# FofanovLab/mtsv_tools

Hardware: AMD Instinct MI355X
Metric: reads/sec (whole node), 150bp reads vs MG-index (higher is better)
Workload: dtype u32/i16

## Files before the change

include/mtsv_amd.h:

```cpp
#ifndef MTSV_AMD_H
#define MTSV_AMD_H

#include <stddef.h>
#include <stdint.h>

#ifdef __cplusplus
extern "C" {
#endif

#define MTSV_OK 0
#define MTSV_E_ARG (-1)
#define MTSV_E_IO (-2)
#define MTSV_E_FORMAT (-3)
#define MTSV_E_DEVICE (-4)
#define MTSV_E_LIMIT (-5)
#define MTSV_E_NOMEM (-6)

typedef struct mtsv_index mtsv_index;
typedef struct mtsv_batch mtsv_batch;

typedef struct {
    double edit_rate;
    uint32_t seed_size;
    uint32_t seed_interval;
    double min_seed;
    uint64_t max_hits;
    uint64_t tune_max_hits;
    int64_t max_assignments;
    int64_t max_candidates;
} mtsv_params;

typedef struct {
    uint64_t read;
    uint32_t tax_id;
    uint32_t gi;
    uint32_t edit;
    uint8_t strand;
    uint8_t _pad[3];
    uint64_t offset;
} mtsv_hit;

typedef struct {
    uint64_t n;
    uint64_t n_bins;
    uint32_t occ_k;
    uint64_t sa_s;
    uint64_t file_bytes;
    uint64_t device_bytes;
    uint32_t kmer_k;
    uint32_t sa_full;
} mtsv_index_info_t;

#define MTSV_N_STAGES 8
typedef struct {
    float stage_ms[MTSV_N_STAGES];
    uint64_t n_reads;
    uint64_t n_seed_slots;
    uint64_t n_seed_hits;
    uint64_t lf_steps;
    uint64_t n_candidates;
    uint64_t n_verified;
    uint64_t window_bytes;
    uint64_t n_hits;
    uint64_t n_passes;
    uint64_t n_rounds;
    uint64_t n_lanes;
    uint64_t sw_cell_pairs;
    float sw_prefilter_ms;
    float sw_sweep_ms;
    uint64_t n_sw_passed;
    float sw_diag_ms;
    float sw_bound_ms;
    float edit_ms;
    uint64_t myers_columns;
    uint64_t n_sw_bound_refuted;
} mtsv_batch_stats;

const char *mtsv_last_error(void);
const char *mtsv_version(void);
void mtsv_params_default(mtsv_params *p);

int mtsv_device_count(void);

int mtsv_index_load(const char *path, mtsv_index **out);
int mtsv_index_build(uint64_t n_seqs, const uint32_t *tax_ids, const uint32_t *gis,
                     const uint8_t *const *seqs, const uint64_t *seq_lens, uint32_t occ_k,
                     uint64_t sa_s, int n_threads, mtsv_index **out);
int mtsv_index_build_fasta(const char *fasta_path, uint32_t occ_k, uint64_t sa_s, int n_threads,
                           mtsv_index **out);
int mtsv_set_build_device(int hip_device);
int mtsv_index_write(const mtsv_index *ix, const char *path);
int mtsv_index_info(const mtsv_index *ix, mtsv_index_info_t *info);
void mtsv_index_free(mtsv_index *ix);

#define MTSV_DEV_DEFAULT 0u
#define MTSV_DEV_SAMPLED_SA_ONLY 1u
#define MTSV_DEV_NO_KMER_TABLE 2u
int mtsv_index_to_device(mtsv_index *ix, int hip_device, uint32_t flags);

int mtsv_bin_batch(mtsv_index *ix, int hip_device, const uint8_t *bases, const uint64_t *read_off,
                   uint64_t n_reads, const mtsv_params *params, mtsv_hit **hits, uint64_t *n_hits);
void mtsv_hits_free(mtsv_hit *hits);
void *mtsv_host_alloc(size_t bytes);
void mtsv_host_free(void *p);
int mtsv_host_register(void *p, size_t bytes);
int mtsv_host_unregister(void *p);
int mtsv_bin_batch_multi(mtsv_index *ix, const int *devices, int n_devices, const uint8_t *bases,
                         const uint64_t *read_off, uint64_t n_reads, const mtsv_params *params,
                         mtsv_hit **hits, uint64_t *n_hits);
int mtsv_bin_batch_chunks(mtsv_index *const *chunks, const int *devices, int n_chunks,
                          const uint8_t *bases, const uint64_t *read_off, uint64_t n_reads,
                          const mtsv_params *params, mtsv_hit **hits, uint64_t *n_hits);
uint64_t mtsv_bin_batch_workspace_reads(uint64_t n_reads);

int mtsv_batch_create(mtsv_index *ix, int hip_device, uint64_t max_reads, uint64_t max_bases,
                      uint64_t max_hits_ws, mtsv_batch **out);
int mtsv_batch_create_lanes(mtsv_index *ix, int hip_device, uint64_t max_reads, uint64_t max_bases,
                            uint64_t max_hits_ws, int lanes, mtsv_batch **out);
int mtsv_batch_reserve_host(mtsv_batch *b, uint64_t n_reads, uint64_t n_bases, uint32_t warm_read_len);
#define MTSV_VERIFY_REFERENCE 0
#define MTSV_VERIFY_EDIT_FIRST 1
int mtsv_batch_set_verify_mode(mtsv_batch *b, int mode);
int mtsv_set_default_verify_mode(int mode);
int mtsv_batch_upload(mtsv_batch *b, const uint8_t *bases, const uint64_t *read_off,
                      uint64_t n_reads);
int mtsv_batch_run(mtsv_batch *b, const mtsv_params *params);
int mtsv_batch_run_host(mtsv_batch *b, const uint8_t *bases, const uint64_t *read_off,
                        uint64_t n_reads, const mtsv_params *params);
int mtsv_batch_run_host_parts(mtsv_batch *b, int n_parts, const uint8_t *const *bases, const uint64_t *const *read_off,
                              const uint64_t *n_reads, const mtsv_params *params);
int mtsv_batch_stats_get(const mtsv_batch *b, mtsv_batch_stats *st);

typedef struct {
    uint32_t tax_id;
    uint32_t _pad;
    uint64_t only_hit, only_best, tied_best, not_best;
} mtsv_taxon_stats;
int mtsv_batch_set_taxa_report(mtsv_batch *b, int on);
int mtsv_batch_taxa_report(mtsv_batch *b, mtsv_taxon_stats **rows, uint64_t *n_rows, uint64_t *total_reads,
                           float *device_ms, int reset);
int mtsv_merge_taxa_reports(const mtsv_taxon_stats *a, uint64_t n_a, const mtsv_taxon_stats *b, uint64_t n_b,
                            mtsv_taxon_stats **out, uint64_t *n_out);
int mtsv_format_taxa_report(const mtsv_taxon_stats *rows, uint64_t n_rows, uint64_t total_reads, char **out,
                            uint64_t *out_len);

#define MTSV_MATCH_OFF 0
#define MTSV_MATCH_WITH_HITS 1
#define MTSV_MATCH_ONLY 2
int mtsv_batch_set_match_flags(mtsv_batch *b, int mode);
int mtsv_batch_match_flags(mtsv_batch *b, uint64_t **words, uint64_t *n_reads, uint64_t *n_matched);
int mtsv_batch_download(mtsv_batch *b, mtsv_hit **hits, uint64_t *n_hits);
void mtsv_batch_free(mtsv_batch *b);

int mtsv_format_results(const mtsv_hit *hits, uint64_t n_hits, const char *ids,
                        const uint64_t *id_off, uint64_t n_reads, int long_format, char **out,
                        uint64_t *out_len);
void mtsv_free(void *p);

uint8_t mtsv_pack_bases(uint8_t *dst, const uint8_t *src, uint64_t first_offset, uint64_t n, uint8_t prev_code);
int mtsv_host_pack_threads(void);

int mtsv_synth_index(uint64_t seed, uint32_t n_taxa, uint32_t gis_per_taxon, uint64_t seq_len,
                     uint32_t occ_k, uint64_t sa_s, int n_threads, mtsv_index **out);
int mtsv_synth_reads(const mtsv_index *ix, uint64_t seed, uint64_t n_reads, uint32_t read_len,
                     uint8_t *bases, uint64_t *read_off);

#ifdef __cplusplus
}
#endif
#endif
```

mtsv_tools_amd/_lib.py:

```python
import ctypes as C
import os

import numpy as np

_HERE = os.path.dirname(os.path.abspath(__file__))


def lib_path():
    return os.environ.get("MTSV_AMD_LIB") or os.path.join(_HERE, "libmtsv_amd.so")


class MtsvError(RuntimeError):
    def __init__(self, code, msg):
        super().__init__(f"mtsv error {code}: {msg}")
        self.code = code


E_ARG, E_IO, E_FORMAT, E_DEVICE, E_LIMIT, E_NOMEM = -1, -2, -3, -4, -5, -6
MATCH_OFF, MATCH_WITH_HITS, MATCH_ONLY = 0, 1, 2


class Params(C.Structure):
    _fields_ = [("edit_rate", C.c_double), ("seed_size", C.c_uint32), ("seed_interval", C.c_uint32),
                ("min_seed", C.c_double), ("max_hits", C.c_uint64), ("tune_max_hits", C.c_uint64),
                ("max_assignments", C.c_int64), ("max_candidates", C.c_int64)]


class IndexInfo(C.Structure):
    _fields_ = [("n", C.c_uint64), ("n_bins", C.c_uint64), ("occ_k", C.c_uint32),
                ("sa_s", C.c_uint64), ("file_bytes", C.c_uint64), ("device_bytes", C.c_uint64),
                ("kmer_k", C.c_uint32), ("sa_full", C.c_uint32)]


N_STAGES = 8
STAGE_NAMES = ("search", "thin_scan", "expand", "locate", "coalesce", "verify", "gather", "total")


class BatchStats(C.Structure):
    _fields_ = [("stage_ms", C.c_float * N_STAGES), ("n_reads", C.c_uint64),
                ("n_seed_slots", C.c_uint64), ("n_seed_hits", C.c_uint64), ("lf_steps", C.c_uint64),
                ("n_candidates", C.c_uint64), ("n_verified", C.c_uint64),
                ("window_bytes", C.c_uint64), ("n_hits", C.c_uint64), ("n_passes", C.c_uint64),
                ("n_rounds", C.c_uint64), ("n_lanes", C.c_uint64), ("sw_cell_pairs", C.c_uint64), ("sw_prefilter_ms", C.c_float),
                ("sw_sweep_ms", C.c_float), ("n_sw_passed", C.c_uint64), ("sw_diag_ms", C.c_float), ("sw_bound_ms", C.c_float),
                ("edit_ms", C.c_float), ("myers_columns", C.c_uint64), ("n_sw_bound_refuted", C.c_uint64)]

    def as_dict(self):
        d = {n: (float(getattr(self, n)) if t is C.c_float else int(getattr(self, n))) for n, t in self._fields_[1:]}
        d["stage_ms"] = {STAGE_NAMES[i]: float(self.stage_ms[i]) for i in range(N_STAGES)}
        return d


HIT_DTYPE = np.dtype({"names": ["read", "tax_id", "gi", "edit", "strand", "offset"],
                      "formats": ["<u8", "<u4", "<u4", "<u4", "u1", "<u8"],
                      "offsets": [0, 8, 12, 16, 20, 24], "itemsize": 32})

TAXON_STATS_DTYPE = np.dtype({"names": ["tax_id", "only_hit", "only_best", "tied_best", "not_best"],
                              "formats": ["<u4", "<u8", "<u8", "<u8", "<u8"],
                              "offsets": [0, 8, 16, 24, 32], "itemsize": 40})

EXPORTS = [
    "mtsv_last_error", "mtsv_version", "mtsv_params_default", "mtsv_device_count",
    "mtsv_index_load", "mtsv_index_build", "mtsv_index_build_fasta", "mtsv_index_write",
    "mtsv_index_info", "mtsv_index_free", "mtsv_set_build_device", "mtsv_index_to_device", "mtsv_bin_batch",
    "mtsv_hits_free", "mtsv_batch_create", "mtsv_batch_upload", "mtsv_batch_run", "mtsv_batch_run_host", "mtsv_batch_run_host_parts",
    "mtsv_batch_stats_get", "mtsv_batch_set_verify_mode", "mtsv_batch_download", "mtsv_batch_free", "mtsv_format_results",
    "mtsv_free", "mtsv_synth_index", "mtsv_synth_reads", "mtsv_bin_batch_workspace_reads",
    "mtsv_bin_batch_multi", "mtsv_bin_batch_chunks", "mtsv_set_default_verify_mode",
    "mtsv_host_alloc", "mtsv_host_free", "mtsv_host_register", "mtsv_host_unregister",
    "mtsv_batch_create_lanes", "mtsv_batch_reserve_host", "mtsv_pack_bases", "mtsv_host_pack_threads",
    "mtsv_batch_set_taxa_report", "mtsv_batch_taxa_report", "mtsv_merge_taxa_reports", "mtsv_format_taxa_report",
    "mtsv_batch_set_match_flags", "mtsv_batch_match_flags",
]

_lib = None


def lib():
    global _lib
    if _lib is None:
        p = lib_path()
        if not os.path.exists(p):
            raise MtsvError(E_DEVICE, f"{p} is missing: run `make -C mtsv_tools_amd/csrc` "
                                      "(or __graft_entry__.build()); there is no fallback path")
        L = C.CDLL(p)
        vp, u64, u32, i32 = C.c_void_p, C.c_uint64, C.c_uint32, C.c_int
        L.mtsv_last_error.restype = C.c_char_p
        L.mtsv_version.restype = C.c_char_p
        L.mtsv_params_default.argtypes = [C.POINTER(Params)]
        L.mtsv_index_load.argtypes = [C.c_char_p, C.POINTER(vp)]
        L.mtsv_index_build.argtypes = [u64, vp, vp, vp, vp, u32, u64, i32, C.POINTER(vp)]
        L.mtsv_index_build_fasta.argtypes = [C.c_char_p, u32, u64, i32, C.POINTER(vp)]
        L.mtsv_index_write.argtypes = [vp, C.c_char_p]
        L.mtsv_index_info.argtypes = [vp, C.POINTER(IndexInfo)]
        L.mtsv_index_free.argtypes = [vp]
        L.mtsv_index_free.restype = None
        L.mtsv_index_to_device.argtypes = [vp, i32, u32]
        L.mtsv_bin_batch.argtypes = [vp, i32, vp, vp, u64, C.POINTER(Params), C.POINTER(vp),
                                     C.POINTER(u64)]
        L.mtsv_hits_free.argtypes = [vp]
        L.mtsv_hits_free.restype = None
        L.mtsv_bin_batch_multi.argtypes = [vp, vp, i32, vp, vp, u64, C.POINTER(Params), C.POINTER(vp), C.POINTER(u64)]
        L.mtsv_bin_batch_chunks.argtypes = [vp, vp, i32, vp, vp, u64, C.POINTER(Params), C.POINTER(vp), C.POINTER(u64)]
        L.mtsv_bin_batch_workspace_reads.argtypes = [u64]
        L.mtsv_bin_batch_workspace_reads.restype = u64
        L.mtsv_batch_create.argtypes = [vp, i32, u64, u64, u64, C.POINTER(vp)]
        L.mtsv_batch_create_lanes.argtypes = [vp, i32, u64, u64, u64, i32, C.POINTER(vp)]
        L.mtsv_batch_reserve_host.argtypes = [vp, u64, u64, u32]
        L.mtsv_pack_bases.argtypes = [vp, vp, u64, u64, C.c_uint8]
        L.mtsv_pack_bases.restype = C.c_uint8
        L.mtsv_batch_upload.argtypes = [vp, vp, vp, u64]
        L.mtsv_batch_run.argtypes = [vp, C.POINTER(Params)]
        L.mtsv_batch_run_host.argtypes = [vp, vp, vp, u64, C.POINTER(Params)]
        L.mtsv_batch_run_host_parts.argtypes = [vp, i32, vp, vp, vp, C.POINTER(Params)]
        L.mtsv_batch_set_verify_mode.argtypes = [vp, i32]
        L.mtsv_batch_stats_get.argtypes = [vp, C.POINTER(BatchStats)]
        L.mtsv_batch_download.argtypes = [vp, C.POINTER(vp), C.POINTER(u64)]
        L.mtsv_batch_free.argtypes = [vp]
        L.mtsv_batch_free.restype = None
        L.mtsv_format_results.argtypes = [vp, u64, C.c_char_p, vp, u64, i32, C.POINTER(vp),
                                          C.POINTER(u64)]
        L.mtsv_free.argtypes = [vp]
        L.mtsv_free.restype = None
        L.mtsv_synth_index.argtypes = [u64, u32, u32, u64, u32, u64, i32, C.POINTER(vp)]
        L.mtsv_synth_reads.argtypes = [vp, u64, u64, u32, vp, vp]
        L.mtsv_host_alloc.argtypes = [C.c_size_t]
        L.mtsv_host_alloc.restype = vp
        L.mtsv_host_free.argtypes = [vp]
        L.mtsv_host_free.restype = None
        L.mtsv_host_register.argtypes = [vp, C.c_size_t]
        L.mtsv_host_unregister.argtypes = [vp]
        L.mtsv_batch_set_taxa_report.argtypes = [vp, i32]
        L.mtsv_batch_taxa_report.argtypes = [vp, C.POINTER(vp), C.POINTER(u64), C.POINTER(u64), C.POINTER(C.c_float), i32]
        L.mtsv_merge_taxa_reports.argtypes = [vp, u64, vp, u64, C.POINTER(vp), C.POINTER(u64)]
        L.mtsv_format_taxa_report.argtypes = [vp, u64, u64, C.POINTER(vp), C.POINTER(u64)]
        L.mtsv_batch_set_match_flags.argtypes = [vp, i32]
        L.mtsv_batch_match_flags.argtypes = [vp, C.POINTER(vp), C.POINTER(u64), C.POINTER(u64)]
        _lib = L
    return _lib


def _check(rc):
    if rc != 0:
        raise MtsvError(rc, lib().mtsv_last_error().decode(errors="replace"))


def version():
    return lib().mtsv_version().decode()


def device_count():
    return lib().mtsv_device_count()


def bin_batch_multi(index, devices, bases, read_off, params=None):
    params = params or default_params()
    bases = np.ascontiguousarray(bases, dtype=np.uint8)
    read_off = np.ascontiguousarray(read_off, dtype=np.uint64)
    dev = (C.c_int * len(devices))(*devices)
    out, n = C.c_void_p(), C.c_uint64()
    _check(lib().mtsv_bin_batch_multi(index.h, dev, len(devices), bases.ctypes.data, read_off.ctypes.data,
                                      len(read_off) - 1, C.byref(params), C.byref(out), C.byref(n)))
    return _hits_from(out, n.value)


def bin_batch_chunks(indexes, devices, bases, read_off, params=None):
    params = params or default_params()
    bases = np.ascontiguousarray(bases, dtype=np.uint8)
    read_off = np.ascontiguousarray(read_off, dtype=np.uint64)
    dev = (C.c_int * len(devices))(*devices)
    hs = (C.c_void_p * len(indexes))(*[ix.h for ix in indexes])
    out, n = C.c_void_p(), C.c_uint64()
    _check(lib().mtsv_bin_batch_chunks(hs, dev, len(indexes), bases.ctypes.data, read_off.ctypes.data,
                                       len(read_off) - 1, C.byref(params), C.byref(out), C.byref(n)))
    return _hits_from(out, n.value)


class HostBuffer:

    def __init__(self, nbytes):
        self.ptr = lib().mtsv_host_alloc(nbytes)
        if not self.ptr:
            raise MtsvError(E_DEVICE, lib().mtsv_last_error().decode(errors="replace"))
        self.array = np.ctypeslib.as_array((C.c_uint8 * max(1, nbytes)).from_address(self.ptr))[:nbytes]

    def close(self):
        if self.ptr:
            self.array = None
            lib().mtsv_host_free(self.ptr)
            self.ptr = None


def pack_bases(bases, first_offset=0, prev_code=0):
    bases = np.ascontiguousarray(bases, dtype=np.uint8)
    n = len(bases)
    out = np.zeros(((first_offset + n + 1) >> 1) - (first_offset >> 1) + 1, dtype=np.uint8)
    last = lib().mtsv_pack_bases(out.ctypes.data, bases.ctypes.data, first_offset, n, prev_code)
    return out[:-1], last


def host_register(arr):
    _check(lib().mtsv_host_register(arr.ctypes.data, arr.nbytes))


def host_unregister(arr):
    _check(lib().mtsv_host_unregister(arr.ctypes.data))


def bin_batch_slice_reads(n_reads):
    return int(lib().mtsv_bin_batch_workspace_reads(n_reads))


def set_build_device(device):
    lib().mtsv_set_build_device.argtypes = [C.c_int]
    _check(lib().mtsv_set_build_device(device))


def default_params(**over):
    p = Params()
    lib().mtsv_params_default(C.byref(p))
    names = {f[0] for f in Params._fields_}
    for k, v in over.items():
        if k not in names:
            raise AttributeError(f"no such parameter: {k}")
        setattr(p, k, -1 if v is None else v)
    return p


def _hits_from(ptr, n):
    try:
        if n == 0:
            return np.zeros(0, dtype=HIT_DTYPE)
        raw = (C.c_ubyte * (n * HIT_DTYPE.itemsize)).from_address(ptr.value)
        return np.frombuffer(raw, dtype=HIT_DTYPE).copy()
    finally:
        lib().mtsv_hits_free(ptr)


class MGIndex:

    def __init__(self, handle):
        self.h = handle

    @classmethod
    def load(cls, path):
        h = C.c_void_p()
        _check(lib().mtsv_index_load(os.fsencode(path), C.byref(h)))
        return cls(h)

    @classmethod
    def build(cls, entries, occ_k=64, sa_s=32, threads=4):
        entries = list(entries)
        n = len(entries)
        tax = np.array([e[0] for e in entries], dtype=np.uint32)
        gi = np.array([e[1] for e in entries], dtype=np.uint32)
        bufs = [C.create_string_buffer(bytes(e[2]), max(len(e[2]), 1)) for e in entries]
        ptrs = (C.c_void_p * max(n, 1))(*[C.addressof(b) for b in bufs])
        lens = np.array([len(e[2]) for e in entries], dtype=np.uint64)
        h = C.c_void_p()
        _check(lib().mtsv_index_build(n, tax.ctypes.data, gi.ctypes.data, ptrs, lens.ctypes.data,
                                      occ_k, sa_s, threads, C.byref(h)))
        return cls(h)

    @classmethod
    def build_fasta(cls, path, occ_k=64, sa_s=32, threads=4):
        h = C.c_void_p()
        _check(lib().mtsv_index_build_fasta(os.fsencode(path), occ_k, sa_s, threads, C.byref(h)))
        return cls(h)

    @classmethod
    def synth(cls, seed, n_taxa, gis_per_taxon, seq_len, occ_k=64, sa_s=32, threads=8):
        h = C.c_void_p()
        _check(lib().mtsv_synth_index(seed, n_taxa, gis_per_taxon, seq_len, occ_k, sa_s, threads,
                                      C.byref(h)))
        return cls(h)

    def write(self, path):
        _check(lib().mtsv_index_write(self.h, os.fsencode(path)))

    def info(self):
        i = IndexInfo()
        _check(lib().mtsv_index_info(self.h, C.byref(i)))
        return {n: int(getattr(i, n)) for n, _ in i._fields_}

    def to_device(self, device=0, flags=0):
        _check(lib().mtsv_index_to_device(self.h, device, flags))

    def bin_batch(self, bases, read_off, params=None, device=0):
        params = params or default_params()
        bases = np.ascontiguousarray(bases, dtype=np.uint8)
        read_off = np.ascontiguousarray(read_off, dtype=np.uint64)
        out, n = C.c_void_p(), C.c_uint64()
        _check(lib().mtsv_bin_batch(self.h, device, bases.ctypes.data, read_off.ctypes.data,
                                    len(read_off) - 1, C.byref(params), C.byref(out), C.byref(n)))
        return _hits_from(out, n.value)

    def close(self):
        if self.h is not None and _lib is not None:
            _lib.mtsv_index_free(self.h)
        self.h = None

    def __del__(self):
        try:
            self.close()
        except Exception:
            pass


class Batch:

    def __init__(self, index, device, max_reads, max_bases, max_hits_ws=0, lanes=0):
        self.index = index
        self.h = C.c_void_p()
        _check(lib().mtsv_batch_create_lanes(index.h, device, max_reads, max_bases, max_hits_ws, lanes,
                                             C.byref(self.h)))

    def reserve_host(self, n_reads, n_bases, warm_read_len=0):
        _check(lib().mtsv_batch_reserve_host(self.h, n_reads, n_bases, warm_read_len))

    def upload(self, bases, read_off):
        bases = np.ascontiguousarray(bases, dtype=np.uint8)
        read_off = np.ascontiguousarray(read_off, dtype=np.uint64)
        _check(lib().mtsv_batch_upload(self.h, bases.ctypes.data, read_off.ctypes.data,
                                       len(read_off) - 1))

    def set_verify_mode(self, mode):
        _check(lib().mtsv_batch_set_verify_mode(self.h, mode))

    def run(self, params=None):
        params = params or default_params()
        _check(lib().mtsv_batch_run(self.h, C.byref(params)))

    def run_host(self, bases, read_off, params=None):
        params = params or default_params()
        bases = np.ascontiguousarray(bases, dtype=np.uint8)
        read_off = np.ascontiguousarray(read_off, dtype=np.uint64)
        _check(lib().mtsv_batch_run_host(self.h, bases.ctypes.data, read_off.ctypes.data, len(read_off) - 1,
                                         C.byref(params)))

    def run_host_parts(self, parts, params=None):
        params = params or default_params()
        keep = [(np.ascontiguousarray(b, dtype=np.uint8), np.ascontiguousarray(o, dtype=np.uint64)) for b, o in parts]
        k = len(keep)
        bp = (C.c_void_p * k)(*[b.ctypes.data for b, _ in keep])
        op = (C.c_void_p * k)(*[o.ctypes.data for _, o in keep])
        nr = (C.c_uint64 * k)(*[len(o) - 1 for _, o in keep])
        _check(lib().mtsv_batch_run_host_parts(self.h, k, bp, op, nr, C.byref(params)))

# ... 101 lines not shown
```

mtsv_tools_amd/csrc/batch.hip:

```cpp
#include <atomic>
#include <chrono>
#include <cmath>
#include <condition_variable>
#include <exception>
#include <mutex>
#include <thread>
#include <cstdio>
#include <cstdlib>
#include <cstring>
#include <stdexcept>
#include <vector>

#include "../../include/mtsv_amd.h"
#include "batch.hpp"
#include "kernels.hpp"

namespace mtsv {

namespace {
template <class F>
void parallel_ranges(uint64_t n, F f) {
    static const int max_nt = [] {
        const char* e = getenv("MTSV_COPY_THREADS");
        return e ? std::max(1, std::min(16, atoi(e))) : 4;
    }();
    const int nt = std::min(max_nt, n >= (32ull << 20) ? 4 : n >= (4ull << 20) ? 2 : 1);
    if (nt == 1) return f(0, n);
    std::vector<std::thread> th;
    const uint64_t chunk = ((n + nt - 1) / nt + 4095) & ~4095ull;
    for (int k = 0; k < nt; k++) {
        uint64_t a = std::min(n, chunk * k), b = std::min(n, chunk * (k + 1));
        if (a < b) th.emplace_back([=] { f(a, b); });
    }
    for (auto& t : th) t.join();
}
double now_s() { return std::chrono::duration<double>(std::chrono::steady_clock::now().time_since_epoch()).count(); }
void parallel_copy(uint8_t* dst, const uint8_t* src, uint64_t n) {
    parallel_ranges(n, [=](uint64_t a, uint64_t b) { memcpy(dst + a, src + a, b - a); });
}

template <class T>
void dev_alloc(T** p, uint64_t count, uint64_t* bytes) {
    uint64_t b = std::max<uint64_t>(count, 1) * sizeof(T);
    HIP_CHECK(hipMalloc((void**)p, b));
    *bytes += b;
}
}

bool host_pinned(const void* p, uint64_t bytes) {
    if (!p || !bytes) return false;
    for (const uint8_t* q : {(const uint8_t*)p, (const uint8_t*)p + bytes - 1}) {
        hipPointerAttribute_t at;
        memset(&at, 0, sizeof at);
        if (hipPointerGetAttributes(&at, q) != hipSuccess) {
            (void)hipGetLastError();
            return false;
        }
        if (at.type != hipMemoryTypeHost) return false;
    }
    return true;
}

void* host_pinned_alloc(uint64_t bytes) {
    void* p = nullptr;
    if (hipHostMalloc(&p, bytes ? bytes : 1, hipHostMallocPortable) != hipSuccess) {
        (void)hipGetLastError();
        return nullptr;
    }
    return p;
}
void host_pinned_free(void* p) {
    if (p && hipHostFree(p) != hipSuccess) (void)hipGetLastError();
}
bool host_pinned_register(void* p, uint64_t bytes) {
    if (hipHostRegister(p, bytes, hipHostRegisterPortable) == hipSuccess) return true;
    (void)hipGetLastError();
    return false;
}
bool host_pinned_unregister(void* p) {
    if (hipHostUnregister(p) == hipSuccess) return true;
    (void)hipGetLastError();
    return false;
}


int g_default_verify_mode = MTSV_VERIFY_REFERENCE;

constexpr uint64_t kLaneMinReads = 32768;
constexpr uint64_t kChunkMaxReads = 4ull << 20;

Batch::Batch(mtsv_index* ix_, DeviceIndex* di_, uint64_t max_reads_, uint64_t max_bases_, uint64_t hit_cap_, Batch* parent_, int lanes_)
    : ix(ix_), di(di_), max_reads(max_reads_), max_bases(max_bases_), hit_cap(hit_cap_), parent(parent_) {
    if (max_reads == 0) max_reads = 1;
    if (max_reads > 0x7fffffffull) throw std::runtime_error("limit: more than 2^31 reads in one batch");
    if (max_bases >= 0xffffffffull) throw std::runtime_error("limit: 4 GiB of bases or more in one batch");
    const uint64_t hit_cap_user = hit_cap;
    if (!parent) {
        n_lanes = 3;
        if (lanes_ > 0) n_lanes = std::min(8, lanes_);
        else if (const char* e = getenv("MTSV_LANES")) n_lanes = std::max(1, std::min(8, atoi(e)));
        if (max_reads < (uint64_t)n_lanes * kLaneMinReads) n_lanes = 1;
    }
    ws_reads = (max_reads + n_lanes - 1) / n_lanes;
    if (!parent && n_lanes > 1) {
        uint64_t cmax = kChunkMaxReads;
        if (const char* e = getenv("MTSV_CHUNK")) cmax = std::max<uint64_t>(kLaneMinReads, strtoull(e, nullptr, 10));
        ws_reads = std::min(ws_reads, cmax);
    }
    if (hit_cap == 0) hit_cap = std::max<uint64_t>(1ull << 20, 32 * ws_reads);
    if (hit_cap > 0xfffffff0ull) hit_cap = 0xfffffff0ull;
    hits_cap = std::max<uint64_t>(1ull << 20, 16 * ws_reads);
    if (const char* e = getenv("MTSV_HITS_CAP")) hits_cap = std::max<uint64_t>(1024, strtoull(e, nullptr, 10));
    HIP_CHECK(hipSetDevice(di->device));
    HIP_CHECK(hipStreamCreateWithFlags(&stream, hipStreamNonBlocking));
    const uint64_t ns = 2 * ws_reads;
    if (!parent) {
        dev_alloc(&d_bases, max_bases + 64, &bytes);
        dev_alloc(&d_read_off, max_reads + 1, &bytes);
        dev_alloc(&d_codes, max_bases + 64, &bytes);
    }
    dev_alloc(&d_strand_hits, ns + 1, &bytes);
    dev_alloc(&d_strand_nseeds, ns, &bytes);
    dev_alloc(&d_strand_off, ns + 1, &bytes);
    dev_alloc(&d_strand_ncand, ns, &bytes);
    dev_alloc(&d_strand_nout, ns + 1, &bytes);
    dev_alloc(&d_heavy_list, 2 * ns, &bytes);
    dev_alloc(&d_out_off, ns + 1, &bytes);
    dev_alloc(&d_tile_sums, (uint64_t)scan_tiles((uint32_t)ns) + 1, &bytes);
    dev_alloc(&d_counters, kCounters, &bytes);
    alloc_hit_workspace();
    dev_alloc(&d_hits, hits_cap, &bytes);
    HIP_CHECK(hipHostMalloc((void**)&h_counters, kCounters * sizeof(uint64_t), hipHostMallocMapped));
    if (const char* e = getenv("MTSV_SW")) sw_pairs = strcmp(e, "packed") != 0;
    if (const char* e = getenv("MTSV_SW_DIAG")) sw_diag = atoi(e) != 0;
    if (const char* e = getenv("MTSV_SW_PREPASS")) sw_prepass = atoi(e) != 0;
    if (const char* e = getenv("MTSV_SW_TOP")) sw_top = atoi(e) != 0;
    if (const char* e = getenv("MTSV_SW_BOUND")) sw_bound = atoi(e) != 0;
    if (const char* e = getenv("MTSV_SW_FUSED")) sw_fused = atoi(e) != 0;
    verify_mode = g_default_verify_mode;
    if (const char* e = getenv("MTSV_VERIFY")) verify_mode = !strcmp(e, "edit_first") ? 1 : 0;
    for (auto& e : ev) HIP_CHECK(hipEventCreate(&e));
    for (int k = 1; k < n_lanes; k++) {
        extra.emplace_back(new Batch(ix, di, ws_reads, 0, hit_cap_user, this));
        bytes += extra.back()->bytes;
    }
}

Batch::~Batch() {
    extra.clear();
    (void)hipSetDevice(di->device);
    (void)hipStreamSynchronize(stream);
    for (void* p : {(void*)d_bases, (void*)d_read_off, (void*)d_seed_lo, (void*)d_seed_cnt, (void*)d_seed_pre, (void*)d_strand_hits,
                    (void*)d_strand_nseeds, (void*)d_strand_off, (void*)d_strand_ncand, (void*)d_worklist,
                    (void*)d_strand_nout, (void*)d_out_off, (void*)d_tile_sums, (void*)d_counters, (void*)d_hit_row,
                    (void*)d_hit_ref, (void*)d_hit_q, (void*)d_hit_key, (void*)d_cand_tmp, (void*)d_cand, (void*)d_out,
                    (void*)d_hits, (void*)d_cand_next, (void*)d_cand_status, (void*)d_heavy_list})
        (void)hipFree(p);
    (void)hipFree(d_codes);
    (void)hipFree(d_strip);
    (void)hipFree(d_planes);
    (void)hipFree(report.d_taxa);
    (void)hipFree(report.d_counts);
    for (auto& e : report_ev)
        if (e) (void)hipEventDestroy(e);
    (void)hipFree(match.d_words);
    for (auto& e : match_ev)
        if (e) (void)hipEventDestroy(e);
    if (h_hits_stage) pinned_hits_release(h_hits_stage);
    if (copy_stream2) (void)hipStreamDestroy(copy_stream2);
    if (copy_stream) {
        (void)hipStreamSynchronize(copy_stream);
        (void)hipStreamDestroy(copy_stream);
    }
    for (auto& ar : arena) {
        (void)hipFree(ar.d_bases);
        (void)hipFree(ar.d_packed);
        (void)hipFree(ar.d_off);
    }
    if (h_off_all) (void)hipHostFree(h_off_all);
    for (auto& hs : h_stage)
        if (hs) (void)hipHostFree(hs);
    for (auto& e : chunk_ev) (void)hipEventDestroy(e);
    (void)hipHostFree(h_counters);
    for (auto& e : ev) (void)hipEventDestroy(e);
    (void)hipStreamDestroy(stream);
}

void Batch::alloc_hit_workspace() {
    dev_alloc(&d_hit_row, hit_cap, &bytes);
    dev_alloc(&d_hit_ref, hit_cap, &bytes);
    dev_alloc(&d_hit_q, hit_cap, &bytes);
    dev_alloc(&d_hit_key, hit_cap, &bytes);
    dev_alloc(&d_cand_tmp, 2 * hit_cap, &bytes);
    dev_alloc(&d_cand, hit_cap, &bytes);
    dev_alloc(&d_out, hit_cap, &bytes);
    dev_alloc(&d_cand_next, hit_cap, &bytes);
    dev_alloc(&d_cand_status, hit_cap, &bytes);
    dev_alloc(&d_worklist, hit_cap, &bytes);
}

void Batch::grow_hit_workspace(uint64_t need) {
    if (getenv("MTSV_TRACE")) fprintf(stderr, "[workspace] seed-hit arrays grow %llu -> %llu entries\n", (unsigned long long)hit_cap, (unsigned long long)need);
    HIP_CHECK(hipStreamSynchronize(stream));
    for (void* p : {(void*)d_hit_row, (void*)d_hit_ref, (void*)d_hit_q, (void*)d_hit_key, (void*)d_cand_tmp, (void*)d_cand,
                    (void*)d_out, (void*)d_cand_next, (void*)d_cand_status, (void*)d_worklist})
        (void)hipFree(p);
    d_hit_row = d_hit_ref = d_hit_q = d_cand_next = d_cand_status = d_worklist = nullptr;
    d_hit_key = d_cand_tmp = nullptr;
    d_cand = d_out = nullptr;
    hit_cap = need;
    alloc_hit_workspace();
}

void Batch::upload(const uint8_t* bases, const uint64_t* read_off, uint64_t n) {
    if (n > max_reads) throw std::runtime_error("arg: batch holds more reads than the workspace was created for");
    const uint64_t first = n ? read_off[0] : 0;
    const uint64_t nb = n ? read_off[n] - first : 0;
    if (nb > max_bases) throw std::runtime_error("arg: batch holds more bases than the workspace was created for");
    h_read_off.resize(n + 1);
    max_len = 0;
    for (uint64_t i = 0; i <= n; i++) {
        if (i && read_off[i] < read_off[i - 1]) throw std::runtime_error("arg: read_off is not ascending");
        h_read_off[i] = (uint32_t)(read_off[i] - first);
        if (i) max_len = std::max(max_len, h_read_off[i] - h_read_off[i - 1]);
    }
    if (n == 0) h_read_off[0] = 0;
    HIP_CHECK(hipSetDevice(di->device));
    if (nb) HIP_CHECK(hipMemcpyAsync(d_bases, bases + first, nb, hipMemcpyHostToDevice, stream));
    HIP_CHECK(hipMemcpyAsync(d_read_off, h_read_off.data(), (n + 1) * 4, hipMemcpyHostToDevice, stream));
    HIP_CHECK(hipStreamSynchronize(stream));
    n_reads = n;
    n_hits_total = 0;
    total_hits = 0;
    segments.clear();
}

void Batch::reset_lane() {
    HIP_CHECK(hipSetDevice(di->device));
    memset(&stats, 0, sizeof stats);
    memset(stage_acc, 0, sizeof stage_acc);
    sw_ms_acc = 0;
    sweep_ms_acc = diag_ms_acc = bound_ms_acc = edit_ms_acc = 0;
    sw_passed_acc = 0;
    n_hits_total = 0;
    HIP_CHECK(hipMemsetAsync(d_counters, 0, kCounters * sizeof(uint64_t), stream));
    HIP_CHECK(hipEventRecord(ev[8], stream));
}

void Batch::finish_lane() {
    HIP_CHECK(hipEventRecord(ev[9], stream));
    launch_publish(stream, d_counters, h_counters, kCounters);
    HIP_CHECK(hipStreamSynchronize(stream));
    HIP_CHECK(hipEventElapsedTime(&stage_acc[7], ev[8], ev[9]));
    if (getenv("MTSV_TRACE")) fprintf(stderr, "[lane] last pass: %llu strands of 13..64 seed hits (or more than 4 candidates) to k_coalesce_mid, %llu heavier ones\n",
                                      (unsigned long long)(h_counters[15] & 0xffffffffull), (unsigned long long)(h_counters[1] >> 32));
    if (getenv("MTSV_TRACE")) fprintf(stderr, "[lane] k_coalesce_heavy: %llu strands walked by runs, %llu by the wavefront walk (a run too long)\n",
                                      (unsigned long long)(h_counters[kCtrHeavyWalk] & 0xffffffffull), (unsigned long long)(h_counters[kCtrHeavyWalk] >> 32));
    stats.sw_cell_pairs = h_counters[14];
    stats.sw_prefilter_ms = sw_ms_acc;
    stats.sw_sweep_ms = sweep_ms_acc;
    stats.sw_diag_ms = diag_ms_acc;
    stats.sw_bound_ms = bound_ms_acc;
    stats.edit_ms = edit_ms_acc;
    stats.myers_columns = h_counters[19];
    stats.n_sw_bound_refuted = h_counters[20];
    stats.n_sw_passed = sw_passed_acc + h_counters[21];
    stats.lf_steps = h_counters[2];
    stats.n_candidates = h_counters[3];
    stats.n_verified = h_counters[4];
    stats.window_bytes = h_counters[5];
}

void Batch::begin_run(const mtsv_params& p, uint64_t read_base) {
    if (!(p.edit_rate >= 0.0 && p.edit_rate <= 1.0)) throw std::runtime_error("arg: edit_rate must be within [0, 1]");
    if (!(p.min_seed >= 0.0) || !std::isfinite(p.min_seed)) throw std::runtime_error("arg: min_seed must be finite and >= 0");
    if (p.seed_size == 0 || p.seed_interval == 0) throw std::runtime_error("arg: seed_size and seed_interval must be > 0");
    segments.clear();
    total_hits = 0;
    lanes_used = 1;
    staged_valid = false;
    run_t0 = now_s();
    reset_lane();
    for (auto& l : extra) {
        l->verify_mode = verify_mode;
        l->sw_pairs = sw_pairs;
        l->sw_diag = sw_diag;
        l->sw_prepass = sw_prepass;
        l->sw_top = sw_top;
        l->sw_bound = sw_bound;
        l->sw_fused = sw_fused;
        l->reset_lane();
    }
    if (match.mode != MTSV_MATCH_OFF) {
        const uint64_t need = (n_reads + 63) / 64;
        if (need > match.cap_words || !match.d_words) {
            (void)hipFree(match.d_words);
            match.d_words = nullptr;
            match.cap_words = 0;
            uint64_t b = 0;
            dev_alloc(&match.d_words, need + need / 16 + 1, &b);
            match.cap_words = need + need / 16;
        }
        match.n_reads = n_reads;
        match.call_base = read_base;
        match.ms = 0;
        match.launches = 0;
        HIP_CHECK(hipMemsetAsync(match.d_words, 0, (match.cap_words + 1) * sizeof(uint64_t), stream));
        HIP_CHECK(hipStreamSynchronize(stream));
    }
}

void Batch::end_run() {
    finish_lane();
    for (auto& l : extra) l->finish_lane();
    const double wall_ms = (now_s() - run_t0) * 1e3;
    bool overlapped = false;
    for (auto& l : extra) {
        if (l->stats.n_passes == 0) continue;
        overlapped = true;
        for (int s = 0; s < 7; s++) stage_acc[s] += l->stage_acc[s];
        stats.n_seed_slots += l->stats.n_seed_slots;
        stats.n_seed_hits += l->stats.n_seed_hits;
        stats.n_passes += l->stats.n_passes;
        stats.n_rounds = std::max(stats.n_rounds, l->stats.n_rounds);
        stats.lf_steps += l->stats.lf_steps;
        stats.n_candidates += l->stats.n_candidates;
        stats.n_verified += l->stats.n_verified;
        stats.window_bytes += l->stats.window_bytes;
        stats.sw_cell_pairs += l->stats.sw_cell_pairs;
        stats.sw_prefilter_ms += l->stats.sw_prefilter_ms;
        stats.sw_sweep_ms += l->stats.sw_sweep_ms;
        stats.sw_diag_ms += l->stats.sw_diag_ms;
        stats.sw_bound_ms += l->stats.sw_bound_ms;
        stats.edit_ms += l->stats.edit_ms;
        stats.myers_columns += l->stats.myers_columns;
        stats.n_sw_bound_refuted += l->stats.n_sw_bound_refuted;
        stats.n_sw_passed += l->stats.n_sw_passed;
    }
    if (overlapped) stage_acc[7] = (float)wall_ms;
    for (int s = 0; s < MTSV_N_STAGES; s++) stats.stage_ms[s] = stage_acc[s];
    stats.n_reads = n_reads;
    stats.n_lanes = lanes_used;
    total_hits = 0;
    for (auto& sg : segments) total_hits += sg.count;
    stats.n_hits = total_hits;
}

void Batch::set_taxa_report(bool on) {
    if (parent) throw std::runtime_error("internal: the taxa report belongs to the workspace's owner");
    if (on && match.mode == MTSV_MATCH_ONLY)
        throw std::runtime_error("arg: the taxa report reads gathered hits and MTSV_MATCH_ONLY gathers none (mtsv_batch_set_match_flags)");
    if (on && !report.d_counts) {
        std::vector<uint32_t>& t = report.h_taxa;
        t.clear();
        for (const Bin& b : ix->host.bins) t.push_back(b.tax_id);
        std::sort(t.begin(), t.end());
        t.erase(std::unique(t.begin(), t.end()), t.end());
        if (t.size() >= (1ull << 30)) throw std::runtime_error("limit: taxa report of 2^30 TaxIDs or more");
        report.n_taxa = (uint32_t)t.size();
        uint32_t dense_max = kReportDenseTaxa;
        if (const char* e = getenv("MTSV_REPORT_DENSE_MAX")) dense_max = (uint32_t)std::min<uint64_t>(strtoull(e, nullptr, 10), kReportDenseTaxa);
        report.dense = report.n_taxa <= dense_max;
        if (const char* e = getenv("MTSV_REPORT_HASH_SLOTS")) {
            const uint64_t want = std::min<uint64_t>(std::max<uint64_t>(strtoull(e, nullptr, 10), 16), kReportHashSlots);
            report.hash_slots = 16;
            while (report.hash_slots * 2 <= want) report.hash_slots *= 2;
        }
        report.trace = getenv("MTSV_TRACE") != nullptr;
        if (report.trace)
            fprintf(stderr, "[report] %u taxa: %s tier (dense up to %u taxa, hash table of %u slots)\n", report.n_taxa,
                    report.dense ? "dense" : "hashed", dense_max, report.hash_slots);
        HIP_CHECK(hipSetDevice(di->device));
        uint64_t b = 0;
        dev_alloc(&report.d_taxa, report.n_taxa, &b);
        dev_alloc(&report.d_counts, 4ull * report.n_taxa + 2, &b);
        if (report.n_taxa) HIP_CHECK(hipMemcpyAsync(report.d_taxa, t.data(), t.size() * 4, hipMemcpyHostToDevice, stream));
        HIP_CHECK(hipMemsetAsync(report.d_counts, 0, (4ull * report.n_taxa + 2) * 8, stream));
        HIP_CHECK(hipStreamSynchronize(stream));
    }
    report.on = on;
}

void Batch::taxa_report(std::vector<mtsv_taxon_stats>& rows, uint64_t* total_reads, float* device_ms, bool reset) {
    if (!report.on) throw std::runtime_error("arg: the taxa report of this workspace is not switched on (mtsv_batch_set_taxa_report)");
    HIP_CHECK(hipSetDevice(di->device));
    const uint64_t n = 4ull * report.n_taxa + 2;
    std::vector<uint64_t> c(n);
    HIP_CHECK(hipMemcpyAsync(c.data(), report.d_counts, n * 8, hipMemcpyDeviceToHost, stream));
    if (reset) HIP_CHECK(hipMemsetAsync(report.d_counts, 0, n * 8, stream));
    HIP_CHECK(hipStreamSynchronize(stream));
    rows.clear();
    for (uint32_t k = 0; k < report.n_taxa; k++) {
        const uint64_t* q = &c[4ull * k];
        if (q[0] | q[1] | q[2] | q[3]) rows.push_back(mtsv_taxon_stats{report.h_taxa[k], 0, q[0], q[1], q[2], q[3]});
    }
    *total_reads = c[n - 2];
    std::lock_guard<std::mutex> lk(report.mu);
    *device_ms = report.ms;
    if (report.trace)
        fprintf(stderr, "[report] %llu kernel launches, %.3f ms, %llu atomic adds on the global counters\n", (unsigned long long)report.launches,
                report.ms, (unsigned long long)c[n - 1]);
    if (reset) report.ms = 0, report.launches = 0;
}

void Batch::set_match_flags(int mode) {
    if (parent) throw std::runtime_error("internal: the match flags belong to the workspace's owner");
    if (mode != MTSV_MATCH_OFF && mode != MTSV_MATCH_WITH_HITS && mode != MTSV_MATCH_ONLY) throw std::runtime_error("arg: bad match-flags mode");
    if (mode == MTSV_MATCH_ONLY && report.on)
        throw std::runtime_error("arg: MTSV_MATCH_ONLY gathers no hits and the taxa report of this workspace, which reads them, is on");
    if (mode != MTSV_MATCH_OFF && match.mode == MTSV_MATCH_OFF) match.n_reads = 0;
    match.trace = getenv("MTSV_TRACE") != nullptr;
    match.mode = mode;
}

void Batch::match_flags(std::vector<uint64_t>& words, uint64_t* n_reads_out, uint64_t* n_matched) {
    if (match.mode == MTSV_MATCH_OFF) throw std::runtime_error("arg: the match flags of this workspace are not switched on (mtsv_batch_set_match_flags)");
    const uint64_t nw = (match.n_reads + 63) / 64;
    words.assign(std::max<uint64_t>(nw, 1), 0);
    *n_reads_out = match.n_reads;
    *n_matched = 0;
    if (!match.n_reads) return;
    HIP_CHECK(hipSetDevice(di->device));
    HIP_CHECK(hipMemcpyAsync(words.data(), match.d_words, nw * 8, hipMemcpyDeviceToHost, stream));
    HIP_CHECK(hipMemcpyAsync(n_matched, match.d_words + match.cap_words, 8, hipMemcpyDeviceToHost, stream));
    HIP_CHECK(hipStreamSynchronize(stream));
    std::lock_guard<std::mutex> lk(match.mu);
    if (match.trace)
        fprintf(stderr, "[match] %llu kernel launches, %.3f ms, %llu of %llu reads matched, %llu bytes of flags to the host\n",
                (unsigned long long)match.launches, match.ms, (unsigned long long)*n_matched, (unsigned long long)match.n_reads,
                (unsigned long long)(nw * 8 + 8));
}

void Batch::run(const mtsv_params& p) {
    begin_run(p);
    run_range(p, d_bases, d_codes, d_read_off, h_read_off.data(), n_reads, max_len, 0);
    end_run();
}

void Batch::run_range(const mtsv_params& p, const uint8_t* raw, uint8_t* sb, const uint32_t* so, const uint32_t* h_off, uint64_t n,
                      uint32_t range_max_len, uint64_t read_base) {
    std::vector<Batch*> ls{this};
    for (auto& l : extra) ls.push_back(l.get());
    uint64_t k = n >= ls.size() * kLaneMinReads ? ls.size() : 1;
    uint64_t per_lane = 2;
    if (const char* e = getenv("MTSV_CHUNKS_PER_LANE")) per_lane = std::max(1, atoi(e));
    uint64_t n_chunks = std::max<uint64_t>(k, (n + ws_reads - 1) / ws_reads);
    if (k > 1 && n >= k * per_lane * kLaneMinReads) n_chunks = std::max(n_chunks, k * per_lane);
    std::vector<uint64_t> bound(n_chunks + 1, n);
    bound[0] = 0;
    while (k > 1 && n_chunks >= 2 * k && (double)n / ((double)n_chunks - (double)(k - 1) / 2.0) > (double)ws_reads) n_chunks++;
    bound.assign(n_chunks + 1, n);
    bound[0] = 0;
    if (k > 1 && n_chunks >= 2 * k) {
        const double per0 = (double)n / ((double)n_chunks - (double)(k - 1) / 2.0);
        uint64_t at = 0;
        for (uint64_t c = 0; c < k; c++) {
            at += (uint64_t)(per0 * (double)(c + 1) / (double)k);
            bound[c + 1] = std::min(at, n);
        }
        const uint64_t rest = n - bound[k], m = n_chunks - k;
        for (uint64_t c = 0; c < m; c++) bound[k + c + 1] = bound[k] + rest * (c + 1) / m;
    } else {
        for (uint64_t c = 0; c < n_chunks; c++) bound[c + 1] = n * (c + 1) / n_chunks;
    }
    for (uint64_t c = 0; c < n_chunks; c++)
        if (bound[c + 1] - bound[c] > ws_reads) throw std::runtime_error("arg: range holds more reads than the workspace was created for");
    k = std::min(k, n_chunks);
    lanes_used = std::max<uint64_t>(lanes_used, k);
    std::vector<Segment> segs(n_chunks);
    std::atomic<uint64_t> next{0};
    auto work = [&](Batch* lane) {
        for (;;) {
            const uint64_t c = next.fetch_add(1);
            if (c >= n_chunks) return;
            const uint64_t a = bound[c], b = bound[c + 1];
            const uint64_t before = lane->n_hits_total;
            if (raw) launch_normalise(lane->stream, raw, sb, h_off[a], h_off[b]);
            lane->run_slice(p, sb, so + a, h_off ? h_off + a : nullptr, b - a, range_max_len, read_base + a);
            segs[c] = Segment{lane, before, lane->n_hits_total - before};
        }
    };
    if (k == 1) {
        work(this);
    } else {
        std::vector<std::exception_ptr> errs(k);
        std::vector<std::thread> th;
        for (uint64_t i = 1; i < k; i++)
            th.emplace_back([&, i] {
                try {
                    HIP_CHECK(hipSetDevice(di->device));
                    work(ls[i]);
                } catch (...) {
                    errs[i] = std::current_exception();
                    next.store(n_chunks);
                }
            });
        try {
            work(this);
        } catch (...) {
            errs[0] = std::current_exception();
            next.store(n_chunks);
        }
        for (auto& t : th) t.join();
        for (auto& e : errs)
            if (e) std::rethrow_exception(e);
    }
    for (auto& sg : segs) segments.push_back(sg);
}

void Batch::run_slice(const mtsv_params& p, const uint8_t* sb, const uint32_t* so, const uint32_t* h_off, uint64_t n_slice,
                      uint32_t slice_max_len, uint64_t read_base) {
    if (slice_max_len > kMaxReadLen)
        throw std::runtime_error("limit: read of " + std::to_string(slice_max_len) + " bases; this build verifies reads up to " +
                                 std::to_string(kMaxReadLen));
    const DevIndexView& v = di->view;
    const uint32_t K = p.seed_size, G = p.seed_interval;
    const bool only_flags = flags_only();
    float* stage_ms = stage_acc;
    const bool mixed = slice_max_len > kMaxRegisterReadLen;
    if (mixed && !h_off) throw std::runtime_error("internal: a slice with long reads needs its host offsets");
    constexpr uint64_t kLongPassSlots = 16ull << 20;

    uint64_t pass_reads = n_slice;
    uint64_t r0 = 0;
    while (r0 < n_slice) {
        uint32_t nr = (uint32_t)std::min<uint64_t>(pass_reads, n_slice - r0);
        uint32_t pass_max_len = slice_max_len;
        bool tiled = false;
        if (mixed) {
            auto len_of = [&](uint64_t i) { return h_off[i + 1] - h_off[i]; };
            tiled = len_of(r0) > kMaxRegisterReadLen;
            uint32_t cnt = 0, ml = 0;
            while (cnt < nr && (len_of(r0 + cnt) > kMaxRegisterReadLen) == tiled) {
                const uint32_t ml2 = std::max(ml, len_of(r0 + cnt));
                if (tiled && cnt && 2ull * (cnt + 1) * (ml2 >= K ? (ml2 - K) / G + 1 : 0) > kLongPassSlots) break;
                ml = ml2;
                cnt++;
            }
            nr = cnt;
            pass_max_len = ml;
        }
        const uint32_t max_ns = pass_max_len >= K ? (pass_max_len - K) / G + 1 : 0;
        const uint32_t nstr = nr * 2;
        const uint64_t slots = (uint64_t)nstr * max_ns;
        if (slots > seed_cap) {
            (void)hipFree(d_seed_lo);
            (void)hipFree(d_seed_cnt);
            (void)hipFree(d_seed_pre);
            d_seed_lo = d_seed_cnt = d_seed_pre = nullptr;
            const uint64_t want = tiled ? slots : std::max<uint64_t>(slots, 2 * ws_reads * (uint64_t)max_ns);
            uint64_t dummy = 0;
            if (getenv("MTSV_TRACE")) fprintf(stderr, "[workspace] seed slot arrays grow %llu -> %llu entries\n", (unsigned long long)seed_cap, (unsigned long long)want);
            dev_alloc(&d_seed_lo, want, &dummy);
            dev_alloc(&d_seed_cnt, want, &dummy);
            dev_alloc(&d_seed_pre, want, &dummy);
            seed_cap = want;
        }
        const bool myers_pass = !tiled && pass_max_len <= 253 && (verify_mode == 1 || (sw_pairs && hit_cap < 0x80000000ull));
        const uint32_t plane_words = myers_pass ? myers_words(pass_max_len) : 0;
        if ((uint64_t)nr * 3 * plane_words > plane_cap) {
            (void)hipFree(d_planes);
            d_planes = nullptr;
            const uint64_t want = std::max<uint64_t>(nr, ws_reads) * 3 * plane_words;
            uint64_t dummy = 0;
            dev_alloc(&d_planes, want, &dummy);
            plane_cap = want;
        }
        HIP_CHECK(hipEventRecord(ev[0], stream));
        const uint32_t listed_cap = (uint32_t)std::min<uint64_t>(slots, std::max<uint64_t>(4096, (uint64_t)((double)slots * listed_share)));
        launch_search(stream, v, sb, so, (uint32_t)r0, nr, max_ns, K, G, d_seed_lo, d_seed_cnt, d_seed_pre, (uint32_t*)(d_counters + 22), listed_cap, di->d_kmer_levels);
        HIP_CHECK(hipEventRecord(ev[1], stream));
        if (max_ns)
            launch_thin(stream, sb, so, (uint32_t)r0, nr, p.edit_rate, p.min_seed, max_ns, K, G, p.max_hits, p.tune_max_hits, d_seed_cnt,
                        d_seed_pre, d_strand_hits, d_strand_nseeds, myers_pass ? d_planes : nullptr, plane_words);
        else {
            HIP_CHECK(hipMemsetAsync(d_strand_hits, 0, (uint64_t)nstr * 4, stream));
            HIP_CHECK(hipMemsetAsync(d_strand_nseeds, 0, (uint64_t)nstr * 4, stream));
        }
        launch_scan(stream, d_strand_hits, nstr, d_tile_sums, d_counters + 0, d_strand_off);
        launch_publish(stream, d_counters, h_counters, 1);
        launch_publish(stream, d_counters + 22, h_counters + 22, 1);
        HIP_CHECK(hipEventRecord(ev[2], stream));
        HIP_CHECK(hipStreamSynchronize(stream));
        {
            const uint64_t n_listed = h_counters[22] & 0xffffffffull;
            const double share = slots ? (double)n_listed / (double)slots : 0.0;
            if (n_listed > listed_cap) {
                listed_share = std::min(1.0, share * 1.25 + 0.01);
                if (getenv("MTSV_TRACE")) fprintf(stderr, "[lane] %llu listed seed slots, grid for %u: pass again\n", (unsigned long long)n_listed, listed_cap);
                continue;
            }
            listed_share = std::min(1.0, std::max(0.02, share * 1.5 + 0.005));
        }
        const uint64_t total_hits = h_counters[0];
        if (total_hits > hit_cap) {
            if (nr > 1) {
                pass_reads = std::max<uint64_t>(1, nr / 2);
                continue;
            }
            if (total_hits > 0xfffffff0ull)
                throw std::runtime_error("device: one read has " + std::to_string(total_hits) + " seed hits, more than 2^32");
            grow_hit_workspace(total_hits);
        }
        stats.n_passes++;
        stats.n_seed_slots += slots;
        stats.n_seed_hits += total_hits;
        launch_expand(stream, v, nstr, max_ns, G, d_seed_lo, d_seed_cnt, d_seed_pre, d_strand_off, d_hit_row, d_hit_ref,
                      d_hit_q);
        HIP_CHECK(hipEventRecord(ev[3], stream));
        if (!v.sa_full)
            launch_locate(stream, v, (uint32_t)total_hits, d_strand_off + nstr, d_hit_row, d_hit_ref,
                          (unsigned long long*)(d_counters + 2));
        HIP_CHECK(hipEventRecord(ev[4], stream));
        HIP_CHECK(hipMemsetAsync(d_counters + 1, 0, 8, stream));
        HIP_CHECK(hipMemsetAsync(d_counters + 7, 0, 8, stream));
        HIP_CHECK(hipMemsetAsync(d_counters + 15, 0, 8, stream));
        launch_coalesce(stream, v, so, (uint32_t)r0, nstr, p.max_candidates, d_strand_off,
                        d_strand_nseeds, d_hit_ref, d_hit_q, d_hit_key, d_cand_tmp, d_cand, d_cand_next,
                        d_cand_status, d_strand_ncand, d_worklist, d_heavy_list, d_counters);
        HIP_CHECK(hipEventRecord(ev[5], stream));
        {
            EvalArgs a;
            a.bases = sb;
            a.read_off = so;
            a.r0 = (uint32_t)r0;
            a.edit_rate = p.edit_rate;
            a.max_candidates = p.max_candidates;
            a.strand_off = d_strand_off;
            a.cand = d_cand;
            a.cand_next = d_cand_next;
            a.cand_status = d_cand_status;
            a.planes = myers_pass ? d_planes : nullptr;
            a.plane_words = plane_words;
            a.out = d_out;
            a.n_verified = (unsigned long long*)(d_counters + 4);
            a.window_bytes = (unsigned long long*)(d_counters + 5);
            a.sw_columns = (unsigned long long*)(d_counters + 14);
            a.worklist = d_worklist;
            a.wl_count = (const uint32_t*)(d_counters + 1);
            a.wl_cursor = (uint32_t*)(d_counters + 7);
            stats.n_rounds = 1;
            if (tiled) {
                HIP_CHECK(hipMemsetAsync(d_counters + 13, 0, sizeof(uint64_t), stream));
                launch_max_window(stream, nstr, d_strand_off, d_strand_ncand, d_cand, (unsigned long long*)(d_counters + 13));
                launch_publish(stream, d_counters + 13, h_counters + 13, 1);
                HIP_CHECK(hipStreamSynchronize(stream));
                const uint32_t strip_len = (uint32_t)std::max<uint64_t>(h_counters[13], 1);
                const uint64_t need = (uint64_t)tiled_groups(total_hits, strip_len) * strip_len;
                if (need > strip_cap) {
                    (void)hipFree(d_strip);
                    d_strip = nullptr;
                    uint64_t dummy = 0;
                    dev_alloc(&d_strip, need, &dummy);
                    strip_cap = need;
                }
                a.strip = d_strip;
                a.strip_len = strip_len;
                launch_evaluate_tiled(stream, v, a, total_hits);
            } else if (verify_mode == 1 && pass_max_len <= 253) {
                launch_edit_myers(stream, v, a, total_hits, pass_max_len);
            } else if (sw_pairs && pass_max_len <= 253 && hit_cap < 0x80000000ull) {
                const bool fused = sw_bound && sw_fused;
                uint32_t* pass_list = (uint32_t*)d_hit_key;
                uint32_t* sweep_list = (uint32_t*)d_hit_key + hit_cap;
                uint32_t* next_lists[2] = {(uint32_t*)d_cand_tmp, (uint32_t*)d_cand_tmp + hit_cap};
                const uint32_t* wl = d_worklist;
                const uint32_t* wl_count = (const uint32_t*)(d_counters + 1);
                uint64_t items = total_hits;
                for (uint32_t round = 0;; round++) {
                    uint64_t* next_slot = d_counters + 11 + (round & 1);
                    HIP_CHECK(hipMemsetAsync(d_counters + 8, 0, 3 * sizeof(uint64_t), stream));
                    HIP_CHECK(hipMemsetAsync(next_slot, 0, sizeof(uint64_t), stream));
                    EvalArgs sw = a;
                    sw.worklist = wl;
                    sw.wl_count = wl_count;
                    sw.wl_cursor = (uint32_t*)(d_counters + 8);
                    sw.wl_reverse = round == 0;
                    sw.counters = d_counters;
                    sw.wl_count_slot = round == 0 ? 1u : 11u + ((round - 1) & 1u);
                    sw.pass_list = pass_list;
                    sw.pass_count = (uint32_t*)(d_counters + 9);
#ifdef MTSV_SW_HIST
                    if (!d_strip) { uint64_t dummy = 0; dev_alloc(&d_strip, 4096, &dummy); strip_cap = 4096; }
                    HIP_CHECK(hipMemsetAsync(d_strip, 0, 768 * 4, stream));
                    sw.strip = d_strip;
#endif
                    if (round == 0) HIP_CHECK(hipEventRecord(ev[10], stream));
                    if (round == 0 && sw_diag && sw_prepass && !fused) {
                        HIP_CHECK(hipMemsetAsync(d_counters + 16, 0, sizeof(uint64_t), stream));
                        launch_sw_diag(stream, v, sw, items, pass_max_len, sweep_list, 16);
                        HIP_CHECK(hipEventRecord(ev[12], stream));
                        sw.worklist = sweep_list;
                        sw.wl_count_slot = 16;
                        sw.wl_reverse = 0;
                    }
                    if (round == 0 && sw_bound) {
                        HIP_CHECK(hipMemsetAsync(d_counters + 17, 0, 2 * sizeof(uint64_t), stream));
                        EvalArgs bd = sw;
                        bd.wl_count = (const uint32_t*)(d_counters + sw.wl_count_slot);
                        bd.wl_cursor = (uint32_t*)(d_counters + 18);
                        bd.und_list = (uint32_t*)d_hit_row;
                        bd.und_slot = 17;
                        bd.myers_ctr = (unsigned long long*)(d_counters + 19);
                        launch_edit_myers(stream, v, bd, items, pass_max_len, fused ? 3 : 2);
                        HIP_CHECK(hipEventRecord(ev[13], stream));
                        sw.worklist = bd.und_list;
                        sw.wl_count_slot = 17;
                        sw.wl_reverse = 0;
                    } else if (round == 0 && sw_diag && sw_prepass && sw_top) {
                        HIP_CHECK(hipMemsetAsync(d_counters + 17, 0, sizeof(uint64_t), stream));
                        sw.und_list = (uint32_t*)d_hit_row;
                        sw.und_slot = 17;
                        launch_sw_pairs(stream, v, sw, items, pass_max_len, false, true);
                        HIP_CHECK(hipMemsetAsync(d_counters + 8, 0, sizeof(uint64_t), stream));
                        sw.worklist = sw.und_list;
                        sw.wl_count_slot = 17;
                    }
                    launch_sw_pairs(stream, v, sw, items, pass_max_len, sw_diag, false, round == 0 && sw_bound);
#ifdef MTSV_SW_HIST
                    {
                        static uint32_t hh[768];
                        HIP_CHECK(hipMemcpyAsync(hh, d_strip, sizeof hh, hipMemcpyDeviceToHost, stream));
                        HIP_CHECK(hipStreamSynchronize(stream));
                        fprintf(stderr, "SWHIST round %u steps/4:", round);
                        for (int i = 0; i < 128; i++) if (hh[i]) fprintf(stderr, " %d:%u", i * 4, hh[i]);
                        fprintf(stderr, "\nSWHIST halves sweeping 0/1/2: %u %u %u\nSWHIST fail best:", hh[128], hh[129], hh[130]);
                        for (int i = 0; i < 256; i++) if (hh[256 + i]) fprintf(stderr, " %d:%u", i, hh[256 + i]);
                        fprintf(stderr, "\nSWHIST pass best:");
                        for (int i = 0; i < 256; i++) if (hh[512 + i]) fprintf(stderr, " %d:%u", i, hh[512 + i]);
                        fprintf(stderr, "\n");
                    }
#endif
                    if (round == 0) HIP_CHECK(hipEventRecord(ev[11], stream));
                    EvalArgs my = a;
                    my.worklist = pass_list;
                    my.wl_count = (const uint32_t*)(d_counters + 9);
                    my.wl_cursor = (uint32_t*)(d_counters + 10);
                    my.next_list = next_lists[round & 1];
                    my.next_count = (uint32_t*)next_slot;
                    my.myers_ctr = (unsigned long long*)(d_counters + 19);
                    launch_edit_myers(stream, v, my, items, pass_max_len, 1);
                    if (round == 0) HIP_CHECK(hipEventRecord(ev[14], stream));
                    launch_publish(stream, next_slot, h_counters + 11, 1);
                    launch_publish(stream, d_counters + 9, h_counters + 9, 1);
                    HIP_CHECK(hipStreamSynchronize(stream));
                    sw_passed_acc += h_counters[9] & 0xffffffffull;
                    if (round == 0) {
                        float ms = 0;
                        HIP_CHECK(hipEventElapsedTime(&ms, ev[10], ev[11]));
                        sw_ms_acc += ms;
                        int from = 10;
                        if (sw_diag && sw_prepass && !fused) {
                            HIP_CHECK(hipEventElapsedTime(&ms, ev[10], ev[12]));
                            diag_ms_acc += ms;
                            from = 12;
                        }
                        if (sw_bound) {
                            HIP_CHECK(hipEventElapsedTime(&ms, ev[from], ev[13]));
                            bound_ms_acc += ms;
                            from = 13;
                        }
                        HIP_CHECK(hipEventElapsedTime(&ms, ev[from], ev[11]));
                        sweep_ms_acc += ms;
                        HIP_CHECK(hipEventElapsedTime(&ms, ev[11], ev[14]));
                        edit_ms_acc += ms;
                    }
                    const uint64_t n_next = h_counters[11] & 0xffffffffull;
                    if (n_next == 0) break;
                    stats.n_rounds++;
                    wl = next_lists[round & 1];
                    wl_count = (const uint32_t*)next_slot;
                    items = n_next;
                }
            } else {
                launch_evaluate(stream, v, a, total_hits, pass_max_len);
            }
            launch_resolve(stream, nstr, p.max_candidates, only_flags ? 1 : p.max_assignments, d_strand_off, d_strand_ncand, d_cand_status,
                           d_out, d_strand_nout);
        }
        HIP_CHECK(hipEventRecord(ev[6], stream));
        uint64_t total_out = 0;
        if (!only_flags) {
            launch_scan(stream, d_strand_nout, nstr, d_tile_sums, d_counters + 6, d_out_off);
            launch_publish(stream, d_counters, h_counters, 8);
            HIP_CHECK(hipStreamSynchronize(stream));
            total_out = h_counters[6];
        }
        if (n_hits_total + total_out > hits_cap) {
            uint64_t ncap = std::max(hits_cap * 2, n_hits_total + total_out);
            DevHit* nh = nullptr;
            uint64_t dummy = 0;
            dev_alloc(&nh, ncap, &dummy);
            if (n_hits_total) HIP_CHECK(hipMemcpyAsync(nh, d_hits, n_hits_total * sizeof(DevHit), hipMemcpyDeviceToDevice, stream));
            HIP_CHECK(hipStreamSynchronize(stream));
            Batch* root = parent ? parent : this;
            std::unique_lock<std::mutex> commit_lk;
            if (root->commit_mu) commit_lk = std::unique_lock<std::mutex>(*root->commit_mu);
            if (root->copy_stream2) HIP_CHECK(hipStreamSynchronize(root->copy_stream2));
            (void)hipFree(d_hits);
            d_hits = nh;
            hits_cap = ncap;
        }
        if (!only_flags) launch_gather(stream, nstr, read_base + r0, d_strand_off, d_strand_nout, d_out_off, d_out, d_hits, n_hits_total);
        HIP_CHECK(hipEventRecord(ev[7], stream));
        TaxaReport& rep = (parent ? parent : this)->report;
        if (rep.on) {
            if (!report_ev[0])
                for (auto& e : report_ev) HIP_CHECK(hipEventCreate(&e));
            HIP_CHECK(hipEventRecord(report_ev[0], stream));
            launch_report(stream, nr, d_strand_nout, d_out_off, d_hits + n_hits_total, rep.d_taxa, rep.n_taxa, rep.dense, rep.hash_slots, rep.d_counts,
                          rep.d_counts + 4ull * rep.n_taxa, rep.trace ? rep.d_counts + 4ull * rep.n_taxa + 1 : nullptr);
            HIP_CHECK(hipEventRecord(report_ev[1], stream));
        }
        MatchFlags& mf = (parent ? parent : this)->match;
        if (mf.mode != MTSV_MATCH_OFF) {
            const uint64_t first_bit = read_base + r0 - mf.call_base;
            if (first_bit + nr > mf.n_reads) throw std::runtime_error("internal: match flags of a pass beyond the run's reads");
            if (!match_ev[0])
                for (auto& e : match_ev) HIP_CHECK(hipEventCreate(&e));
            HIP_CHECK(hipEventRecord(match_ev[0], stream));
            launch_match(stream, nr, d_strand_nout, first_bit, mf.d_words, mf.d_words + mf.cap_words);
            HIP_CHECK(hipEventRecord(match_ev[1], stream));
        }
        HIP_CHECK(hipStreamSynchronize(stream));
        HIP_CHECK(hipGetLastError());
        if (mf.mode != MTSV_MATCH_OFF) {
            float ms = 0;
            HIP_CHECK(hipEventElapsedTime(&ms, match_ev[0], match_ev[1]));
            std::lock_guard<std::mutex> lk(mf.mu);
            mf.ms += ms;
            mf.launches++;
        }
        if (rep.on) {
            float ms = 0;
            HIP_CHECK(hipEventElapsedTime(&ms, report_ev[0], report_ev[1]));
            std::lock_guard<std::mutex> lk(rep.mu);
            rep.ms += ms;
            rep.launches++;
        }
        n_hits_total += total_out;
        for (int s = 0; s < 7; s++) {
            float ms = 0;
            HIP_CHECK(hipEventElapsedTime(&ms, ev[s], ev[s + 1]));
            stage_ms[s] += ms;
        }
        r0 += nr;
    }
}

namespace {
struct PinnedPool {
    std::mutex mu;
    std::vector<std::pair<void*, uint64_t>> free_list;
    std::vector<std::pair<void*, uint64_t>> live;
    static constexpr size_t kKeep = 6;
    void* get(uint64_t bytes, uint64_t* cap) {
        {
            std::lock_guard<std::mutex> lk(mu);
            size_t best = free_list.size();
            for (size_t i = 0; i < free_list.size(); i++)
                if (free_list[i].second >= bytes && (best == free_list.size() || free_list[i].second < free_list[best].second)) best = i;
            if (best != free_list.size()) {
                auto e = free_list[best];
                free_list.erase(free_list.begin() + best);
                live.push_back(e);
                *cap = e.second;
                return e.first;
            }
        }
        void* p = nullptr;
        const uint64_t b = std::max<uint64_t>((bytes + (bytes >> 3) + 4095) & ~4095ull, 1ull << 16);
        HIP_CHECK(hipHostMalloc(&p, b, hipHostMallocPortable));
        std::lock_guard<std::mutex> lk(mu);
        live.emplace_back(p, b);
        *cap = b;
        return p;
    }
    bool put(void* p) {
        std::pair<void*, uint64_t> drop{nullptr, 0};
        {
            std::lock_guard<std::mutex> lk(mu);
            size_t i = 0;
            while (i < live.size() && live[i].first != p) i++;
            if (i == live.size()) return false;
            auto e = live[i];
            live.erase(live.begin() + i);
            free_list.push_back(e);
            if (free_list.size() > kKeep) {
                size_t m = 0;
                for (size_t k = 1; k < free_list.size(); k++)
                    if (free_list[k].second < free_list[m].second) m = k;
                drop = free_list[m];
                free_list.erase(free_list.begin() + m);
            }
        }
        if (drop.first) (void)hipHostFree(drop.first);
        return true;
    }
};
PinnedPool& pool() {
    static PinnedPool* p = new PinnedPool;
    return *p;
}
}

mtsv_hit* pinned_hits_alloc(uint64_t n_hits, uint64_t* cap_hits) {
    uint64_t cap = 0;
    void* p = pool().get(std::max<uint64_t>(n_hits, 1) * sizeof(mtsv_hit), &cap);
    *cap_hits = cap / sizeof(mtsv_hit);
    return (mtsv_hit*)p;
}
bool pinned_hits_release(void* p) { return p && pool().put(p); }

void Batch::run_host(const uint8_t* bases, const uint64_t* read_off, uint64_t n, const mtsv_params& p, uint64_t read_base) {
    const HostPart one{bases, read_off, n};
    run_host_parts(&one, 1, p, read_base);
}

void Batch::host_room(uint64_t n, uint64_t total_bases, bool trace) {
    if (!copy_stream) {
        int prio_low = 0, prio_high = 0;
        HIP_CHECK(hipDeviceGetStreamPriorityRange(&prio_low, &prio_high));
        HIP_CHECK(hipStreamCreateWithPriority(&copy_stream, hipStreamNonBlocking, prio_high));
        HIP_CHECK(hipStreamCreateWithPriority(&copy_stream2, hipStreamNonBlocking, prio_high));
    }
    uint64_t arena_bases = kArenaBases, arena_reads = kArenaReads;
    if (const char* e = getenv("MTSV_ARENA_BASES")) arena_bases = std::max<uint64_t>(1 << 16, strtoull(e, nullptr, 10));
    const bool one_segment = total_bases <= arena_bases && n <= arena_reads;
    {
        const uint64_t want_b = one_segment ? total_bases : arena_bases, want_r = one_segment ? n : std::min(n, arena_reads);
        for (int k = 0; k < (one_segment ? 1 : 2); k++) {
            Arena& ar = arena[k];
            if (ar.cap_bases < want_b || ar.cap_reads < want_r) {
                if (trace) fprintf(stderr, "[run_host] arena %d: %.1f MB of bases, %llu reads\n", k, want_b / 1e6, (unsigned long long)want_r);
                (void)hipFree(ar.d_bases);
                (void)hipFree(ar.d_packed);
                (void)hipFree(ar.d_off);
                ar.d_bases = nullptr;
                ar.d_packed = nullptr;
                ar.d_off = nullptr;
                ar.cap_bases = ar.cap_reads = 0;
                const uint64_t cb = want_b + want_b / 16, cr = want_r + want_r / 16;
                dev_alloc(&ar.d_bases, std::min(cb, arena_bases) + 64, &bytes);
                dev_alloc(&ar.d_packed, std::min(cb, arena_bases) / 2 + 64, &bytes);
                dev_alloc(&ar.d_off, std::min(cr, arena_reads) + 1, &bytes);
                ar.cap_bases = std::min(cb, arena_bases);
                ar.cap_reads = std::min(cr, arena_reads);
            }
        }
    }
    const uint64_t off_need = n + 2 + (one_segment ? 0 : 2 * (total_bases / arena_bases + n / arena_reads) + 8);
    if (h_off_cap < off_need) {
        if (h_off_all) (void)hipHostFree(h_off_all);
        h_off_all = nullptr;
        h_off_cap = off_need + n / 16;
        HIP_CHECK(hipHostMalloc((void**)&h_off_all, h_off_cap * sizeof(uint32_t)));
    }
}

void Batch::reserve_host(uint64_t n, uint64_t n_bases) {
    HIP_CHECK(hipSetDevice(di->device));
    host_room(n, n_bases, getenv("MTSV_TRACE") != nullptr);
    if (!keep_on_device) {
        uint64_t cap = 0;
        mtsv_hit* h = pinned_hits_alloc(n + n / 8, &cap);
        pinned_hits_release(h);
    }
}

void Batch::run_host_parts(const HostPart* parts, int n_parts, const mtsv_params& p, uint64_t read_base) {
    const double t_entry = now_s();
    HIP_CHECK(hipSetDevice(di->device));
    std::vector<Batch*> ls{this};
    for (auto& l : extra) ls.push_back(l.get());
    const bool trace = getenv("MTSV_TRACE") != nullptr;
    struct PartView {
        const uint8_t* bases;
        const uint64_t* off;
        uint64_t n, first, virt;
        bool pinned;
    };
    std::vector<PartView> pv;
    uint64_t n = 0, total_bases = 0;
    for (int k = 0; k < n_parts; k++) {
        const HostPart& hp = parts[k];
        if (!hp.n) continue;
        if (!hp.read_off || hp.read_off[hp.n] < hp.read_off[0]) throw std::runtime_error("arg: read_off is not ascending");
        const uint64_t nb = hp.read_off[hp.n] - hp.read_off[0];
        if (nb && !hp.bases) throw std::runtime_error("arg: null bases");
        const bool pin = nb && host_pinned(hp.bases + hp.read_off[0], nb) && !getenv("MTSV_STAGE_ALWAYS");
        pv.push_back(PartView{hp.bases, hp.read_off, hp.n, n, total_bases, pin});
        n += hp.n;
        total_bases += nb;
    }
    const uint64_t first_base = 0;
    auto part_of = [&](uint64_t r) {
        size_t k = pv.size() - 1;
        while (k > 0 && pv[k].first > r) k--;
        return k;
    };
    auto RO = [&](uint64_t r) {
        if (pv.empty()) return (uint64_t)0;
        const PartView& v = pv[part_of(r)];
        return v.virt + (v.off[r - v.first] - v.off[0]);
    };
    bool any_staged = false, any_direct = false;
    for (auto& v : pv) (v.pinned ? any_direct : any_staged) = true;
    const bool direct = !any_staged;
    if (trace) fprintf(stderr, "[run_host] input %s%s\n", direct ? "page-locked: copied from the caller's buffer" : "pageable: staged",
                       any_staged && any_direct ? " (some parts page-locked)" : "");

    host_room(n, total_bases, trace);
    constexpr uint64_t kChunkMax = 32ull << 20, kChunkMin = 4ull << 20;
    static std::atomic<int> host_runs{0};
    struct HostRun {
        std::atomic<int>& c;
        const int mine;
        explicit HostRun(std::atomic<int>& c_) : c(c_), mine(++c_) {}
        ~HostRun() { c--; }
    } host_run{host_runs};
    const bool packed = !getenv("MTSV_H2D_PLAIN") && pack_threads() >= kPackWorthwhile && host_run.mine == 1;
    if ((packed || !direct) && !h_stage[0])
        for (auto& hs : h_stage) HIP_CHECK(hipHostMalloc((void**)&hs, kChunkMax + 64));

    struct Chunk {
        uint64_t begin = 0, end = 0;
        uint32_t max_len = 0, seg = 0;
        hipEvent_t ev = nullptr;
        bool complete = false;
    };
    struct Range {
        uint64_t begin = 0, end = 0;
        bool done = false;
        Batch* lane = nullptr;
        uint64_t hit_off = 0, hit_cnt = 0;
    };
    std::mutex mu;
    std::condition_variable cv;
    std::vector<Chunk> chunks;
    std::vector<uint64_t> seg_begin{0};
    uint64_t n_complete = 0;
    bool issued_all = n == 0;
    std::vector<Range> ranges;
    uint64_t next_read = 0;
    uint64_t next_commit = 0;
    uint64_t done_prefix = 0;
    int busy_lanes = 0;
    bool abort = false;
    std::exception_ptr first_err;
    auto fail = [&](std::exception_ptr e) {
        std::lock_guard<std::mutex> lk(mu);
        if (!first_err) first_err = e;
        abort = true;
        cv.notify_all();
    };
    auto event_for = [&](size_t k) {
        while (chunk_ev.size() <= k) {
            hipEvent_t e;
            HIP_CHECK(hipEventCreateWithFlags(&e, hipEventDisableTiming));
            chunk_ev.push_back(e);
        }
        return chunk_ev[k];
    };

    n_reads = n;
    max_len = 0;
    if (trace) fprintf(stderr, "[run_host] entered; begin_run at %.2f ms\n", (now_s() - t_entry) * 1e3);
    begin_run(p, read_base);
    staged_hits = 0;
    if (!h_hits_stage && !keep_on_device && !flags_only()) {
        h_hits_stage = pinned_hits_alloc(last_total_hits ? last_total_hits + last_total_hits / 64 : n + n / 8, &h_hits_cap);
    }
    if (trace) fprintf(stderr, "[run_host] result array of %llu hits ready at %.2f ms\n", (unsigned long long)h_hits_cap, (now_s() - t_entry) * 1e3);
    const uint64_t n_lanes_used = n >= ls.size() * kLaneMinReads ? ls.size() : 1;
    lanes_used = n_lanes_used;

    auto watcher = [&]() {
        try {
            HIP_CHECK(hipSetDevice(di->device));
            size_t c = 0;
            for (;;) {
                size_t upto;
                bool last;
                std::vector<hipEvent_t> evs;
                {
                    std::lock_guard<std::mutex> lk(mu);
                    if (abort) return;
                    upto = chunks.size();
                    last = issued_all;
                    for (size_t i = c; i < upto; i++) evs.push_back(chunks[i].ev);
                }
                const size_t c0 = c;
                while (c < upto) {
                    const hipError_t q = hipEventQuery(evs[c - c0]);
                    if (q == hipSuccess) c++;
                    else if (q == hipErrorNotReady) break;
                    else throw_hip(q, "hipEventQuery(chunk)", __FILE__, __LINE__);
                }
                if (c != c0) {
                    {
                        std::lock_guard<std::mutex> lk(mu);
                        n_complete = c;
                    }
                    cv.notify_all();
                }
                if (last && c == upto) return;
                std::this_thread::sleep_for(std::chrono::microseconds(20));
            }
        } catch (...) {
            fail(std::current_exception());
        }
    };
    auto feeder = [&]() {
        try {
            HIP_CHECK(hipSetDevice(di->device));
            uint64_t r = 0, seg = 0, seg_first_base = first_base, seg_first_read = 0;
            uint64_t chunk_bytes = kChunkMin;
            size_t k = 0;
            uint8_t prev_code = 0;
            while (r < n) {
                uint64_t e = r;
                {
                    uint64_t lo = r + 1, hi = n;
                    hi = pv[part_of(r)].first + pv[part_of(r)].n;
                    const uint64_t lim = RO(r) + chunk_bytes;
                    if (RO(hi) > lim) {
                        while (lo < hi) {
                            const uint64_t mid = (lo + hi + 1) / 2;
// ... 285 lines not shown
```

mtsv_tools_amd/csrc/batch.hpp:

```cpp
#pragma once
#include <memory>
#include <mutex>
#include <vector>

#include "../../include/mtsv_amd.h"
#include "host_pack.hpp"
#include "dev_index.hpp"
#include "kernels.hpp"

namespace mtsv {

struct Batch {
    mtsv_index* ix;
    DeviceIndex* di;
    hipStream_t stream = nullptr, copy_stream2 = nullptr;
    mtsv_hit* h_hits_stage = nullptr;
    uint64_t h_hits_cap = 0, staged_hits = 0, last_total_hits = 0;
    bool staged_valid = false;
    struct Arena {
        uint8_t* d_bases = nullptr;
        uint8_t* d_packed = nullptr;
        uint32_t* d_off = nullptr;
        uint64_t cap_bases = 0, cap_reads = 0;
    };
    static constexpr uint64_t kArenaBases = 3ull << 30;
    static constexpr uint64_t kArenaReads = 1ull << 30;
    Arena arena[2];
    uint32_t* h_off_all = nullptr;
    uint64_t h_off_cap = 0;
    static constexpr int kStage = 4;
    uint8_t* h_stage[kStage] = {};
    hipStream_t copy_stream = nullptr;
    std::vector<hipEvent_t> chunk_ev;
    std::mutex* commit_mu = nullptr;
    uint64_t max_reads, max_bases, hit_cap, hits_cap = 0;
    uint64_t bytes = 0;
    Batch* parent = nullptr;
    std::vector<std::unique_ptr<Batch>> extra;
    int n_lanes = 1;
    uint64_t ws_reads = 0;
    struct Segment {
        Batch* lane;
        uint64_t offset, count;
    };
    std::vector<Segment> segments;
    uint64_t total_hits = 0;
    double run_t0 = 0;
    uint64_t lanes_used = 1;

    uint8_t* d_codes = nullptr;
    uint8_t* d_bases = nullptr;
    uint32_t* d_read_off = nullptr;
    uint32_t *d_seed_lo = nullptr, *d_seed_cnt = nullptr, *d_seed_pre = nullptr;
    uint64_t seed_cap = 0;
    uint32_t *d_strand_hits = nullptr, *d_strand_nseeds = nullptr, *d_strand_off = nullptr, *d_strand_ncand = nullptr,
             *d_worklist = nullptr, *d_strand_nout = nullptr, *d_out_off = nullptr;
    uint64_t* d_tile_sums = nullptr;
    uint64_t* d_counters = nullptr;
    uint32_t *d_hit_row = nullptr, *d_hit_ref = nullptr, *d_hit_q = nullptr;
    uint64_t *d_hit_key = nullptr, *d_cand_tmp = nullptr;
    uint4 *d_cand = nullptr, *d_out = nullptr;
    uint32_t *d_cand_next = nullptr, *d_cand_status = nullptr, *d_heavy_list = nullptr;
    DevHit* d_hits = nullptr;
    uint2* d_strip = nullptr;
    uint64_t strip_cap = 0;
    uint32_t* d_planes = nullptr;
    uint64_t plane_cap = 0;
    uint64_t* h_counters = nullptr;
    hipEvent_t ev[15];
    float sw_ms_acc = 0, sweep_ms_acc = 0, diag_ms_acc = 0, bound_ms_acc = 0, edit_ms_acc = 0;
    uint64_t sw_passed_acc = 0;

    std::vector<uint32_t> h_read_off;
    uint32_t max_len = 0;
    static constexpr int kCounters = 25;
    double listed_share = 0.125;
    bool sw_diag = true;
    bool sw_top = true;
    bool sw_bound = true;
    bool sw_fused = true;
    bool sw_prepass = true;
    bool sw_pairs = true;
    int verify_mode = 0;
    uint64_t n_reads = 0;
    uint64_t n_hits_total = 0;
    mtsv_batch_stats stats{};
    float stage_acc[MTSV_N_STAGES] = {0};

    Batch(mtsv_index* ix, DeviceIndex* di, uint64_t max_reads, uint64_t max_bases, uint64_t hit_cap, Batch* parent = nullptr, int lanes = 0);
    ~Batch();
    Batch(const Batch&) = delete;
    Batch& operator=(const Batch&) = delete;

    void upload(const uint8_t* bases, const uint64_t* read_off, uint64_t n);
    void run(const mtsv_params& p);
    void run_host(const uint8_t* bases, const uint64_t* read_off, uint64_t n, const mtsv_params& p, uint64_t read_base = 0);
    struct HostPart {
        const uint8_t* bases;
        const uint64_t* read_off;
        uint64_t n;
    };
    void run_host_parts(const HostPart* parts, int n_parts, const mtsv_params& p, uint64_t read_base = 0);
    void reserve_host(uint64_t n, uint64_t n_bases);
    void download(mtsv_hit** hits, uint64_t* n);
    void download_into(mtsv_hit* dst, uint64_t n);
    bool keep_on_device = false;

    struct TaxaReport {
        bool on = false;
        bool dense = true;
        uint32_t hash_slots = kReportHashSlots;
        uint32_t n_taxa = 0;
        uint32_t* d_taxa = nullptr;
        uint64_t* d_counts = nullptr;
        bool trace = false;
        uint64_t launches = 0;
        std::vector<uint32_t> h_taxa;
        std::mutex mu;
        float ms = 0;
    };
    TaxaReport report;
    hipEvent_t report_ev[2] = {nullptr, nullptr};
    void set_taxa_report(bool on);
    struct MatchFlags {
        int mode = MTSV_MATCH_OFF;
        uint64_t* d_words = nullptr;
        uint64_t cap_words = 0;
        uint64_t n_reads = 0;
        uint64_t call_base = 0;
        bool trace = false;
        std::mutex mu;
        float ms = 0;
        uint64_t launches = 0;
    };
    MatchFlags match;
    hipEvent_t match_ev[2] = {nullptr, nullptr};
    bool flags_only() const { return (parent ? parent : this)->match.mode == MTSV_MATCH_ONLY; }
    void set_match_flags(int mode);
    void match_flags(std::vector<uint64_t>& words, uint64_t* n_reads, uint64_t* n_matched);
    void taxa_report(std::vector<mtsv_taxon_stats>& rows, uint64_t* total_reads, float* device_ms, bool reset);

   private:
    void begin_run(const mtsv_params& p, uint64_t read_base = 0);
    void reset_lane();
    void stage_reserve(uint64_t n_hits_needed);
    void host_room(uint64_t n, uint64_t total_bases, bool trace);
    void finish_lane();
    void alloc_hit_workspace();
    void grow_hit_workspace(uint64_t need);
    void run_range(const mtsv_params& p, const uint8_t* raw, uint8_t* sb, const uint32_t* so, const uint32_t* h_off, uint64_t n,
                   uint32_t range_max_len, uint64_t read_base);
    void run_slice(const mtsv_params& p, const uint8_t* sb, const uint32_t* so, const uint32_t* h_off, uint64_t n_slice,
                   uint32_t slice_max_len, uint64_t read_base);
    void end_run();
};

extern int g_default_verify_mode;

mtsv_hit* pinned_hits_alloc(uint64_t n_hits, uint64_t* cap_hits);
bool pinned_hits_release(void* p);
void* host_pinned_alloc(uint64_t bytes);
void host_pinned_free(void* p);
bool host_pinned_register(void* p, uint64_t bytes);
bool host_pinned_unregister(void* p);
bool host_pinned(const void* p, uint64_t bytes);

}

struct mtsv_batch {
    mtsv::Batch impl;
    template <class... A>
    explicit mtsv_batch(A&&... a) : impl(std::forward<A>(a)...) {}
};
```

mtsv_tools_amd/csrc/k_coalesce.hip:

```cpp
#include <cstring>

#include "kernels_common.hpp"

namespace mtsv {

namespace {

__device__ inline uint64_t wave_bitonic_sort(uint64_t key) {
    const uint32_t lane = lane_id();
    for (uint32_t k = 2; k <= kWave; k <<= 1)
        for (uint32_t j = k >> 1; j > 0; j >>= 1) {
            uint64_t other = __shfl_xor(key, j);
            bool up = (lane & k) == 0;
            bool lower = (lane & j) == 0;
            key = (lower == up) ? min(key, other) : max(key, other);
        }
    return key;
}

template <class V>
__device__ inline uint32_t find_bin(const V& ix, uint32_t site) {
    const uint32_t k = site >> ix.bin_lut_shift;
    uint32_t lo = ix.bin_lut[k], hi = ix.bin_lut[k + 1];
    while (lo < hi) {
// ... 524 lines not shown
        bool to_mid = nh > (uint32_t)(LISTED ? HITS : kLaneHitsSecond) && nh <= (uint32_t)kWave;
        const bool heavy = nh > (uint32_t)kWave;
        uint32_t gnc = 0;
        uint32_t cs[kLaneCands], ce[kLaneCands], cb[kLaneCands], cn[kLaneCands], ct[kLaneCands];
#pragma unroll
        for (int k = 0; k < kLaneCands; k++) cs[k] = ce[k] = cb[k] = cn[k] = ct[k] = 0;
        bool hopeless = false;
        if (nh >= 1 && nh <= (uint32_t)HITS) {
            const uint32_t ns_raw = a.strand_nseeds[rs];
            hopeless = (ns_raw & kHopeless) != 0;
            const StrandGeom gg = strand_geom(a.read_off, r0 + (rs >> 1), ns_raw);
            uint64_t key[HITS];
#pragma unroll
            for (int i = 0; i < HITS; i++)
                key[i] = (uint32_t)i < nh ? ((uint64_t)a.hit_ref[o + i] << 32) | a.hit_q[o + i] : ~0ull;
#define MTSV_CX(I, J)                      \
    {                                      \
        const uint64_t lo_ = key[I] < key[J] ? key[I] : key[J], hi_ = key[I] < key[J] ? key[J] : key[I]; \
        key[I] = lo_;                      \
        key[J] = hi_;                      \
    }
            if (HITS == 12) {
                MTSV_SORT12(MTSV_CX)
            } else {
                MTSV_SORT16(MTSV_CX)
            }
#undef MTSV_CX
            bool have = false;
            uint32_t w_s = 0, w_e = 0, w_b = 0, w_n = 0, w_t = 0;
            uint32_t cur_b = 0xffffffffu;
            DevBin cur{0, 0, 0, 0};
            auto flush = [&]() {
                if (have && w_n >= gg.min_seeds) {
#pragma unroll
                    for (int k = 0; k < kLaneCands; k++)
                        if (gnc == (uint32_t)k) {
                            cs[k] = w_s;
                            ce[k] = w_e;
                            cb[k] = w_b;
                            cn[k] = w_n;
                            ct[k] = w_t;
                        }
                    gnc++;
                }
            };
            if (LISTED) {
#pragma unroll
                for (int i = 0; i < HITS; i++) walk_keys[LISTED ? i : 0][LISTED ? threadIdx.x : 0] = key[i];
            }
            auto walk_step = [&](uint64_t key_i) {
                    const uint32_t site = (uint32_t)(key_i >> 32), q = (uint32_t)key_i;
                    if (cur_b == 0xffffffffu || site >= cur.end) {
                        cur_b = min(find_bin(ix, site), ix.n_bins - 1);
                        cur = ix.bins[cur_b];
                    }
                    uint32_t ws, we;
                    const bool ok = candidate_window(site, q, cur, gg.L, gg.ED, &ws, &we);
                    const bool merge = have && ok && cur_b == w_b && ((w_s <= ws && ws < w_e) || (w_s < we && we <= w_e));
                    if (merge) {
                        w_s = min(w_s, ws);
                        w_e = max(w_e, we);
                        w_n++;
                    } else {
                        flush();
                        have = ok;
                        w_s = ws;
                        w_e = we;
                        w_b = cur_b;
                        w_n = 1;
                        w_t = cur.tax_id;
                    }
            };
            if (LISTED) {
#pragma unroll 1
                for (uint32_t i = 0; i < nh; i++) walk_step(walk_keys[LISTED ? i : 0][LISTED ? threadIdx.x : 0]);
            } else {
#pragma unroll
                for (int i = 0; i < HITS; i++)
                    if ((uint32_t)i < nh) walk_step(key[i]);
            }
            flush();
            if (gnc > (uint32_t)kLaneCands) {
                to_mid = true;
                gnc = 0;
            }
        }
        {
            const unsigned long long bm = __ballot(to_mid), bh = __ballot(heavy);
            if (!LISTED) {
                const unsigned long long bs = __ballot(to_second);
                if (bs) {
                    if (to_second) second_buf[n_second + __popcll(bs & ((1ull << lane) - 1))] = rs;
                    n_second += (uint32_t)__popcll(bs);
                    if (n_second > kMidFlush) flush_second();
                }
            }
            if (bm) {
                if (to_mid) mid_buf[n_mid + __popcll(bm & ((1ull << lane) - 1))] = rs;
                n_mid += (uint32_t)__popcll(bm);
                if (n_mid > kMidFlush) flush_mid();
            }
            if (bh) {
                if (heavy) heavy_buf[n_heavy + __popcll(bh & ((1ull << lane) - 1))] = rs;
                n_heavy += (uint32_t)__popcll(bh);
                if (n_heavy > kHeavyFlush) flush_heavy();
            }
        }
        const bool mine = nh >= 1 && nh <= (uint32_t)HITS && !to_mid;
        uint32_t rank[kLaneCands], nxt[kLaneCands];
        bool first[kLaneCands];
#pragma unroll
        for (int k = 0; k < kLaneCands; k++) {
            rank[k] = 0;
#pragma unroll
            for (int j = 0; j < kLaneCands; j++)
                if (j != k && (uint32_t)j < gnc) rank[k] += (cn[j] > cn[k]) || (cn[j] == cn[k] && j < k);
        }
#pragma unroll
        for (int k = 0; k < kLaneCands; k++) {
            nxt[k] = 0xffffffffu;
            first[k] = (uint32_t)k < gnc;
#pragma unroll
            for (int j = 0; j < kLaneCands; j++)
                if (j != k && (uint32_t)j < gnc && ct[j] == ct[k]) {
                    if (rank[j] > rank[k] && rank[j] < nxt[k]) nxt[k] = rank[j];
                    if (rank[j] < rank[k]) first[k] = false;
                }
        }
        uint32_t n_emit = 0;
        if (mine) {
            cand_sum += gnc;
            if (hopeless) {
                a.strand_ncand[rs] = 0;
                ver_sum += min(gnc, maxc);
#pragma unroll
                for (int k = 0; k < kLaneCands; k++)
                    if ((uint32_t)k < gnc && rank[k] < maxc) win_sum += ce[k] - cs[k];
            } else {
                a.strand_ncand[rs] = gnc;
#pragma unroll
                for (int k = 0; k < kLaneCands; k++)
                    if ((uint32_t)k < gnc) {
                        a.cand[o + rank[k]] = make_uint4(cs[k], ce[k], cb[k], rs);
                        a.cand_next[o + rank[k]] = nxt[k];
                        a.cand_status[o + rank[k]] = 0;
                        n_emit += first[k] && rank[k] < maxc;
                    }
            }
        }
        {
            uint32_t incl = n_emit;
#pragma unroll
            for (int d = 1; d < kWave; d <<= 1) {
                const uint32_t up = (uint32_t)__shfl_up((int)incl, d);
                if (lane >= (uint32_t)d) incl += up;
            }
            const uint32_t total = (uint32_t)__shfl((int)incl, kWave - 1);
            uint32_t at = pend + incl - n_emit;
            if (n_emit) {
#pragma unroll
                for (int k = 0; k < kLaneCands; k++)
                    if ((uint32_t)k < gnc && first[k] && rank[k] < maxc) pend_buf[at++] = o + rank[k];
            }
            pend += total;
            if (pend > kPendFlush) flush_pend();
        }
    }
    if (pend) flush_pend();
    if (n_mid) flush_mid();
    if (!LISTED && n_second) flush_second();
    if (n_heavy) flush_heavy();
    for (int d = 32; d > 0; d >>= 1) {
        cand_sum += __shfl_down(cand_sum, d);
        ver_sum += __shfl_down(ver_sum, d);
        win_sum += __shfl_down(win_sum, d);
    }
    if (lane == 0 && cand_sum) atomicAdd(co_n_cand(a), cand_sum);
    if (lane == 0 && ver_sum) {
        atomicAdd(co_n_cand(a) + 1, ver_sum);
        atomicAdd(co_n_cand(a) + 2, win_sum);
    }
}

__device__ __attribute__((noinline)) uint32_t coalesce_mid_strand(const DevIndexView& ix, const CoalesceArgs& a, uint32_t rs, uint32_t o,
                                                                    uint32_t nh, uint32_t* pend_buf, uint32_t& pend) {
    const uint32_t lane = lane_id();
    const uint32_t ns_raw = a.strand_nseeds[rs];
    const bool hopeless = (ns_raw & kHopeless) != 0;
    const StrandGeom g = strand_geom(a.read_off, a.r0 + (rs >> 1), ns_raw);
    uint32_t nc = 0;
    uint64_t key = lane < nh ? ((uint64_t)a.hit_ref[o + lane] << 32) | a.hit_q[o + lane] : ~0ull;
    key = wave_bitonic_sort(key);
    uint32_t site = (uint32_t)(key >> 32), q = (uint32_t)key;
    uint32_t b = 0, ws = 0, we = 0;
    bool ok = false;
    if (lane < nh) {
        b = min(find_bin(ix, site), ix.n_bins - 1);
        DevBin bin = ix.bins[b];
        ok = candidate_window(site, q, bin, g.L, g.ED, &ws, &we);
    }
    Walk w{false, 0, 0, 0, 0};
    uint32_t ms = 0, me = 0, mb = 0, mn = 0;
    for (uint32_t i = 0; i < nh; i++) {
        uint32_t wsi = (uint32_t)__shfl((int)ws, (int)i), wei = (uint32_t)__shfl((int)we, (int)i);
        uint32_t bi = (uint32_t)__shfl((int)b, (int)i);
        bool oki = (uint32_t)__shfl((int)ok, (int)i) != 0;
        bool merge = w.have && oki && bi == w.b && ((w.s <= wsi && wsi < w.e) || (w.s < wei && wei <= w.e));
        if (merge) {
            w.s = min(w.s, wsi);
            w.e = max(w.e, wei);
            w.n++;
        } else {
            if (w.have && w.n >= g.min_seeds) {
                if (lane == nc) { ms = w.s; me = w.e; mb = w.b; mn = w.n; }
                nc++;
            }
            w.have = oki;
            w.s = wsi; w.e = wei; w.b = bi; w.n = 1;
        }
    }
    if (w.have && w.n >= g.min_seeds) {
        if (lane == nc) { ms = w.s; me = w.e; mb = w.b; mn = w.n; }
        nc++;
    }
    uint32_t rank = 0;
    for (uint32_t j = 0; j < nc; j++) {
        uint32_t nj = (uint32_t)__shfl((int)mn, (int)j);
        rank += (nj > mn) || (nj == mn && j < lane);
    }
    uint32_t tax = lane < nc ? ix.bins[mb].tax_id : 0;
    uint32_t nxt = 0xffffffffu;
    bool first = lane < nc;
    for (uint32_t j = 0; j < nc; j++) {
        uint32_t tj = (uint32_t)__shfl((int)tax, (int)j), rj = (uint32_t)__shfl((int)rank, (int)j);
        if (tj == tax && rj > rank && rj < nxt) nxt = rj;
        if (tj == tax && rj < rank) first = false;
    }
    if (hopeless) {
        unsigned long long wsum = (lane < nc && rank < a.maxc) ? me - ms : 0;
        for (int d = 32; d > 0; d >>= 1) wsum += __shfl_down(wsum, d);
        if (lane == 0) {
            a.strand_ncand[rs] = 0;
            atomicAdd(co_n_cand(a) + 1, (unsigned long long)min(nc, a.maxc));
            atomicAdd(co_n_cand(a) + 2, wsum);
        }
        return nc;
    }
    if (lane < nc) {
        a.cand[o + rank] = make_uint4(ms, me, mb, rs);
        a.cand_next[o + rank] = nxt;
        a.cand_status[o + rank] = 0;
    }
    if (lane == 0) a.strand_ncand[rs] = nc;
    {
        bool emit = first && rank < a.maxc;
        unsigned long long em = __ballot(emit);
        uint32_t m = __popcll(em);
        if (pend + m > kWave) {
            uint32_t base = 0;
            if (lane == 0) base = atomicAdd(co_wl_count(a), pend);
            base = __builtin_amdgcn_readfirstlane(base);
            if (lane < pend) a.worklist[base + lane] = pend_buf[lane];
            pend = 0;
        }
        if (emit) pend_buf[pend + __popcll(em & ((1ull << lane) - 1))] = o + rank;
        pend += m;
    }
    return nc;
}

__global__ __launch_bounds__(256) void k_coalesce_mid(DevIndexView ix, CoalesceArgs a) {
    __shared__ uint32_t pend_all[256 / kWave][kWave];
    uint32_t* pend_buf = pend_all[threadIdx.x / kWave];
    const uint32_t lane = lane_id();
    const uint32_t wave = (blockIdx.x * blockDim.x + threadIdx.x) / kWave;
    const uint32_t n_waves = gridDim.x * blockDim.x / kWave;
    const uint32_t n_list = *co_mid_count(a);
    uint32_t pend = 0;
    unsigned long long cand_sum = 0;
    for (uint32_t h = wave; h < n_list; h += n_waves) {
        const uint32_t rs = a.heavy_list[h];
        const uint32_t o = a.strand_off[rs];
        const uint32_t nh = __builtin_amdgcn_readfirstlane(a.strand_off[rs + 1] - o);
        const uint32_t nc = coalesce_mid_strand(ix, a, rs, o, nh, pend_buf, pend);
        if (lane == 0) cand_sum += nc;
    }
    if (pend) {
        uint32_t base = 0;
        if (lane == 0) base = atomicAdd(co_wl_count(a), pend);
        base = __builtin_amdgcn_readfirstlane(base);
        wave_mem_sync();
        if (lane < pend) a.worklist[base + lane] = pend_buf[lane];
    }
    for (int d = 32; d > 0; d >>= 1) cand_sum += __shfl_down(cand_sum, d);
    if (lane == 0 && cand_sum) atomicAdd(co_n_cand(a), cand_sum);
}

}

void launch_coalesce(hipStream_t s, const DevIndexView& ix, const uint32_t* read_off, uint32_t r0, uint32_t n_strands,
                     int64_t max_candidates, const uint32_t* strand_off,
                     const uint32_t* strand_nseeds, const uint32_t* hit_ref, const uint32_t* hit_q, uint64_t* hit_key,
                     uint64_t* cand_tmp, uint4* cand, uint32_t* cand_next, uint32_t* cand_status,
                     uint32_t* strand_ncand, uint32_t* worklist, uint32_t* heavy_list, uint64_t* counters) {
    uint32_t* wl_count = reinterpret_cast<uint32_t*>(counters + 1);
    uint32_t* heavy_count = wl_count + 1;
    unsigned long long* n_cand_total = reinterpret_cast<unsigned long long*>(counters + 3);
    uint32_t blocks = std::max<uint32_t>(1, std::min<uint32_t>(std::min<uint32_t>(cdiv(n_strands, 16), std::max<uint32_t>(cdiv(n_strands, 4 * 256), 256)), 256 * 8));
    CoalesceArgs c;
    c.read_off = read_off;
    c.r0 = r0;
    c.n_strands = n_strands;
    c.maxc = rank_bound(max_candidates);
    c.strand_off = strand_off;
    c.strand_nseeds = strand_nseeds;
    c.hit_ref = hit_ref;
    c.hit_q = hit_q;
    c.cand = cand;
    c.cand_next = cand_next;
    c.cand_status = cand_status;
    c.strand_ncand = strand_ncand;
    c.worklist = worklist;
    c.heavy_list = heavy_list;
    c.counters = counters;
    hipLaunchKernelGGL((k_coalesce<kLaneHitsFirst, false>), dim3(blocks), dim3(256), 0, s, ix, c);
    hipLaunchKernelGGL((k_coalesce<kLaneHitsSecond, true>), dim3(std::min<uint32_t>(std::max<uint32_t>(n_strands / 8192, 8), 512)), dim3(256), 0, s, ix, c);
    hipLaunchKernelGGL(k_coalesce_mid, dim3(std::min<uint32_t>(std::max<uint32_t>(n_strands / 2048, std::min<uint32_t>(std::max<uint32_t>(n_strands / 256, 1), 128)), 1024)), dim3(256), 0, s, ix, c);
    HeavyArgs a;
    a.read_off = read_off;
    a.r0 = r0;
    a.maxc = rank_bound(max_candidates);
    a.strand_off = strand_off;
    a.strand_nseeds = strand_nseeds;
    a.hit_ref = hit_ref;
    a.hit_q = hit_q;
    a.hit_key = hit_key;
    a.cand_tmp = cand_tmp;
    a.cand = cand;
    a.cand_next = cand_next;
    a.cand_status = cand_status;
    a.strand_ncand = strand_ncand;
    a.worklist = worklist;
    a.wl_count = wl_count;
    a.n_cand_total = n_cand_total;
    const dim3 hgrid(std::min<uint32_t>(std::max<uint32_t>(n_strands / 64, 1), 2048));
    const char* hw = getenv("MTSV_HEAVY_WALK");
    const bool serial_walk = hw && !strcmp(hw, "serial");
    if (serial_walk || ix.n_bins >= 0x80000000u) {
        hipLaunchKernelGGL((k_coalesce_heavy<kHeavyKeysSmall, false>), hgrid, dim3(256), 0, s, ix, a, heavy_list, n_strands, heavy_count);
    } else {
        (void)hipMemsetAsync(counters + kCtrHeavyTicket, 0, sizeof(uint64_t), s);
        hipLaunchKernelGGL((k_coalesce_heavy<kHeavyKeysSmall, true>), hgrid, dim3(256), 0, s, ix, a, heavy_list, n_strands, heavy_count);
    }
    hipLaunchKernelGGL((k_coalesce_heavy<kHeavyKeys, false>), dim3(std::min<uint32_t>(hgrid.x, 512)), dim3(256), 0, s, ix, a, heavy_list, n_strands, heavy_count);
}

namespace {
__global__ __launch_bounds__(256) void k_max_window(uint32_t n_strands, const uint32_t* __restrict__ strand_off,
                                                    const uint32_t* __restrict__ strand_ncand, const uint4* __restrict__ cand,
                                                    unsigned long long* __restrict__ out) {
    const uint32_t rs = blockIdx.x * blockDim.x + threadIdx.x;
    uint32_t m = 0;
    if (rs < n_strands) {
        const uint32_t o = strand_off[rs], nc = strand_ncand[rs];
        for (uint32_t i = 0; i < nc; i++) {
            const uint4 c = cand[o + i];
            m = max(m, c.y - c.x);
        }
    }
    for (int d = 32; d > 0; d >>= 1) m = max(m, (uint32_t)__shfl_down((int)m, d));
    if (lane_id() == 0 && m) atomicMax(out, (unsigned long long)m);
}
}

void launch_max_window(hipStream_t s, uint32_t n_strands, const uint32_t* strand_off, const uint32_t* strand_ncand,
                       const uint4* cand, unsigned long long* out) {
    hipLaunchKernelGGL(k_max_window, dim3(cdiv(n_strands, 256)), dim3(256), 0, s, n_strands, strand_off, strand_ncand, cand, out);
}

}
```

mtsv_tools_amd/csrc/k_seed.hip:

```cpp
#include "kernels_common.hpp"

namespace mtsv {

namespace {

__device__ inline uint32_t fast_code(uint32_t ch);
__global__ __launch_bounds__(256) void k_normalise(const uint8_t* src, uint8_t* dst, uint64_t lo, uint64_t hi) {
    const uint64_t i = (lo & ~15ull) + ((uint64_t)blockIdx.x * blockDim.x + threadIdx.x) * 16;
    if (i >= hi) return;
    if (i < lo || i + 16 > hi) {
        const uint64_t a = i < lo ? lo : i, b = i + 16 > hi ? hi : i + 16;
        for (uint64_t q = a; q < b; q++) dst[q] = (uint8_t)fast_code(src[q]);
        return;
    }
    uint4 v = *reinterpret_cast<const uint4*>(src + i);
    uint32_t w[4] = {v.x, v.y, v.z, v.w};
#pragma unroll
    for (int k = 0; k < 4; k++) {
        uint32_t o = 0;
#pragma unroll
        for (int q = 0; q < 4; q++) o |= fast_code((w[k] >> (8 * q)) & 0xffu) << (8 * q);
        w[k] = o;
    }
    *reinterpret_cast<uint4*>(dst + i) = make_uint4(w[0], w[1], w[2], w[3]);
// ... 368 lines not shown
    if (i >= *slow_count) return;
    search_slot(ix, bases, read_off, r0, max_ns, K, G, slow_list[i], seed_lo, seed_cnt, levels);
}


__global__ __launch_bounds__(256) void k_thin(const uint8_t* __restrict__ bases, const uint32_t* __restrict__ read_off,
                                              uint32_t r0, uint32_t n_reads, double edit_rate, double min_seed,
                                              uint32_t max_ns, uint32_t K, uint32_t G, uint64_t max_hits,
                                              uint64_t tune_max_hits, uint32_t* __restrict__ seed_cnt,
                                              uint32_t* __restrict__ seed_pre, uint32_t* __restrict__ strand_hits,
                                              uint32_t* __restrict__ strand_nseeds, uint32_t* __restrict__ planes,
                                              uint32_t plane_words) {
    uint32_t rs = blockIdx.x * blockDim.x + threadIdx.x;
    if (rs >= n_reads * 2) return;
    uint32_t r = r0 + (rs >> 1);
    const uint32_t b0 = read_off[r];
    uint32_t L = read_off[r + 1] - b0;
    uint32_t ns = n_seeds_of(L, K, G);
    uint64_t next_offset = 0, seed_interval = G;
    uint32_t total = 0, nseeds = 0;
    uint32_t* cnt = seed_cnt + (uint64_t)rs * max_ns;
    uint32_t* pre = seed_pre + (uint64_t)rs * max_ns;
    for (uint32_t j = 0; j < ns; j++) {
        uint64_t offset = (uint64_t)j * G;
        const uint32_t raw = cnt[j];
        const uint32_t c = raw == kSeedAtPos ? 1u : raw;
        if (offset < next_offset) {
            if (c) cnt[j] = 0;
            continue;
        }
        if (c == 0) continue;
        if ((uint64_t)c > max_hits) {
            cnt[j] = 0;
            continue;
        }
        if ((uint64_t)c > tune_max_hits) {
            seed_interval *= 2;
            next_offset = offset + seed_interval;
        }
        pre[j] = total;
        total += c;
        nseeds++;
    }
    {
        const bool need = total != 0;
        const int other_need = __shfl_xor((int)need, 1);
        const bool pair_need = need || other_need != 0;
        const uint32_t ED = (uint32_t)ceil((double)L * edit_rate);
        bool hopeless = 2ull * ED > (uint64_t)L;
        uint32_t nn = 0;
        if (pair_need) {
            const uint4* b128 = reinterpret_cast<const uint4*>(bases);
            const uint32_t q0 = b0 >> 4, q1 = (b0 + L + 15) >> 4;
            const uint32_t half = rs & 1, sh = b0 & 15u, nw = (L + 31) >> 5;
            uint32_t* img = planes ? planes + ((uint64_t)(rs >> 1) * plane_words) * 3 : nullptr;
            uint32_t a0 = 0, a1 = 0, an = 0;
            constexpr uint32_t kAhead = 3;
            for (uint32_t i0 = 0; i0 <= nw; i0 += kAhead) {
              uint4 vb[kAhead];
#pragma unroll
              for (uint32_t u = 0; u < kAhead; u++) {
                  const uint32_t q = q0 + 2 * (i0 + u) + half;
                  vb[u] = make_uint4(0, 0, 0, 0);
                  if (i0 + u <= nw && q < q1) vb[u] = b128[q];
              }
#pragma unroll
              for (uint32_t u = 0; u < kAhead; u++) {
                const uint32_t i = i0 + u;
                if (i > nw) break;
                const uint4 v = vb[u];
                uint32_t h01 = 0, hn = 0;
                {
                    const uint32_t c0 = (v.x & 0x07070707u) | ((v.y & 0x07070707u) << 4);
                    const uint32_t c1 = (v.z & 0x07070707u) | ((v.w & 0x07070707u) << 4);
                    auto gather = [](uint32_t y) {
                        y &= 0x11111111u;
                        y |= y >> 7;
                        y |= y >> 14;
                        return y & 0xffu;
                    };
                    h01 = gather(c0) | (gather(c1) << 8) | (gather(c0 >> 1) << 16) | (gather(c1 >> 1) << 24);
                    hn = gather(c0 >> 2) | (gather(c1 >> 2) << 8);
                }
                const uint32_t o01 = (uint32_t)__builtin_amdgcn_update_dpp(0, (int)h01, 0xB1, 0xf, 0xf, false);
                const uint32_t on = (uint32_t)__builtin_amdgcn_update_dpp(0, (int)hn, 0xB1, 0xf, 0xf, false);
                const uint32_t lo01 = half ? o01 : h01, hi01 = half ? h01 : o01;
                const uint32_t c0 = (lo01 & 0xffffu) | (hi01 << 16), c1 = (lo01 >> 16) | (hi01 & 0xffff0000u);
                const uint32_t cn = half ? (on | (hn << 16)) : (hn | (on << 16));
                if (i && ((i - 1) & 1) == half) {
                    const uint32_t w = i - 1, left = L - 32 * w;
                    const uint32_t m = left >= 32 ? 0xffffffffu : (1u << left) - 1u;
                    const uint32_t w0 = __builtin_amdgcn_alignbit(c0, a0, sh) & m, w1 = __builtin_amdgcn_alignbit(c1, a1, sh) & m,
                                   wn = __builtin_amdgcn_alignbit(cn, an, sh) & m;
                    nn += __popc(wn);
                    if (img) {
                        img[3 * w] = w0;
                        img[3 * w + 1] = w1;
                        img[3 * w + 2] = wn;
                    }
                }
                a0 = c0;
                a1 = c1;
                an = cn;
              }
            }
        }
        nn += (uint32_t)__shfl_xor((int)nn, 1);
        hopeless = hopeless || nn > ED;
        const double ms = floor((double)nseeds * min_seed);
        const uint32_t min_seeds = ms < 1.0 ? 1u : (ms > 65535.0 ? 65535u : (uint32_t)ms);
        nseeds = min_seeds | (ED << 16) | ((need && hopeless) ? kHopeless : 0u);
    }
    strand_hits[rs] = total;
    strand_nseeds[rs] = nseeds;
}

constexpr int kScanThreads = 256;
constexpr int kScanItems = 8;
constexpr int kScanTile = kScanThreads * kScanItems;

__device__ inline uint32_t wave_incl_scan(uint32_t v) {
    for (int d = 1; d < kWave; d <<= 1) {
        uint32_t o = __shfl_up(v, d);
        if ((int)lane_id() >= d) v += o;
    }
    return v;
}

__global__ __launch_bounds__(kScanThreads) void k_scan_tile_sums(const uint32_t* __restrict__ in, uint32_t n,
                                                                 uint64_t* __restrict__ tile_sums) {
    __shared__ uint32_t ws[kScanThreads / kWave];
    uint32_t base = blockIdx.x * kScanTile + threadIdx.x * kScanItems;
    uint32_t s = 0;
    for (int i = 0; i < kScanItems; i++)
        if (base + i < n) s += in[base + i];
    for (int d = 32; d > 0; d >>= 1) s += __shfl_down(s, d);
    if (lane_id() == 0) ws[threadIdx.x / kWave] = s;
    __syncthreads();
    if (threadIdx.x == 0) {
        uint64_t t = 0;
        for (int w = 0; w < kScanThreads / kWave; w++) t += ws[w];
        tile_sums[blockIdx.x] = t;
    }
}

__global__ __launch_bounds__(1024) void k_scan_sums(uint64_t* __restrict__ tile_sums, uint32_t n_tiles,
                                                    uint64_t* __restrict__ total) {
    __shared__ uint64_t buf[1024];
    __shared__ uint64_t carry;
    if (threadIdx.x == 0) carry = 0;
    __syncthreads();
    for (uint32_t base = 0; base < n_tiles; base += 1024) {
        uint32_t i = base + threadIdx.x;
        uint64_t v = i < n_tiles ? tile_sums[i] : 0;
        buf[threadIdx.x] = v;
        __syncthreads();
        for (int d = 1; d < 1024; d <<= 1) {
            uint64_t o = threadIdx.x >= (uint32_t)d ? buf[threadIdx.x - d] : 0;
            __syncthreads();
            buf[threadIdx.x] += o;
            __syncthreads();
        }
        uint64_t incl = buf[threadIdx.x];
        uint64_t c = carry;
        if (i < n_tiles) tile_sums[i] = c + incl - v;
        __syncthreads();
        if (threadIdx.x == 1023) carry = c + incl;
        __syncthreads();
    }
    if (threadIdx.x == 0) *total = carry;
}

__global__ __launch_bounds__(kScanThreads) void k_scan_apply(const uint32_t* __restrict__ in, uint32_t n,
                                                             const uint64_t* __restrict__ tile_sums,
                                                             const uint64_t* __restrict__ total,
                                                             uint32_t* __restrict__ out) {
    __shared__ uint32_t ws[kScanThreads / kWave];
    uint32_t base = blockIdx.x * kScanTile + threadIdx.x * kScanItems;
    uint32_t v[kScanItems];
    uint32_t s = 0;
    for (int i = 0; i < kScanItems; i++) {
        v[i] = base + i < n ? in[base + i] : 0;
        s += v[i];
    }
    uint32_t incl = wave_incl_scan(s);
    if (lane_id() == kWave - 1) ws[threadIdx.x / kWave] = incl;
    __syncthreads();
    uint32_t wbase = 0;
    for (uint32_t w = 0; w < threadIdx.x / kWave; w++) wbase += ws[w];
    uint32_t run = (uint32_t)tile_sums[blockIdx.x] + wbase + incl - s;
    for (int i = 0; i < kScanItems; i++) {
        if (base + i < n) out[base + i] = run;
        run += v[i];
    }
    if (blockIdx.x == 0 && threadIdx.x == 0) out[n] = (uint32_t)*total;
}

__global__ __launch_bounds__(256) void k_expand(DevIndexView ix, uint64_t n_slots, uint32_t max_ns, uint32_t G,
                                                const uint32_t* __restrict__ seed_lo,
                                                const uint32_t* __restrict__ seed_cnt,
                                                const uint32_t* __restrict__ seed_pre,
                                                const uint32_t* __restrict__ strand_off,
                                                uint32_t* __restrict__ hit_row, uint32_t* __restrict__ hit_ref,
                                                uint32_t* __restrict__ hit_q) {
    uint64_t slot = (uint64_t)blockIdx.x * blockDim.x + threadIdx.x;
    const uint32_t raw = slot < n_slots ? seed_cnt[slot] : 0;
    const bool at_pos = raw == kSeedAtPos;
    const uint32_t c = at_pos ? 1u : raw;
    uint32_t o = 0, l = 0, q = 0;
    if (c) {
        const uint32_t rs = (uint32_t)(slot / max_ns), j = (uint32_t)(slot % max_ns);
        o = strand_off[rs] + seed_pre[slot];
        l = seed_lo[slot];
        q = j * G;
    }
    constexpr uint32_t kOwn = 16;
    if (at_pos) {
        hit_ref[o] = l;
        hit_q[o] = q;
    } else if (c && c <= kOwn) {
        for (uint32_t i = 0; i < c; i++) {
            if (ix.sa_full) hit_ref[o + i] = ix.sa_full[l + i];
            else hit_row[o + i] = l + i;
            hit_q[o + i] = q;
        }
    }
    unsigned long long big = __ballot(c > kOwn);
    const uint32_t lane = lane_id();
    while (big) {
        const int src = __ffsll((long long)big) - 1;
        big &= big - 1;
        const uint32_t cs = __builtin_amdgcn_readlane(c, src), os = __builtin_amdgcn_readlane(o, src);
        const uint32_t ls = __builtin_amdgcn_readlane(l, src), qs = __builtin_amdgcn_readlane(q, src);
        for (uint32_t i = lane; i < cs; i += kWave) {
            if (ix.sa_full) hit_ref[os + i] = ix.sa_full[ls + i];
            else hit_row[os + i] = ls + i;
            hit_q[os + i] = qs;
        }
    }
}

constexpr uint32_t kLocateChunk = 512;

__global__ __launch_bounds__(256) void k_locate(DevIndexView ix, const uint32_t* __restrict__ total_hits,
                                                const uint32_t* __restrict__ hit_row,
                                                uint32_t* __restrict__ hit_ref, unsigned long long* __restrict__ lf_steps) {
    const uint32_t total = *total_hits;
    const uint32_t lane = lane_id();
    const uint32_t wave = (blockIdx.x * blockDim.x + threadIdx.x) / kWave;
    const uint32_t n_waves = gridDim.x * blockDim.x / kWave;
    unsigned long long my_steps = 0;
    for (uint64_t cbase = (uint64_t)wave * kLocateChunk; cbase < total; cbase += (uint64_t)n_waves * kLocateChunk) {
        uint32_t next = (uint32_t)cbase;
        const uint32_t end = (uint32_t)min((uint64_t)total, cbase + kLocateChunk);
        bool active = false;
        uint32_t idx = 0, row = 0, steps = 0;
        for (;;) {
            unsigned long long need = __ballot(!active);
            uint32_t take = next + __popcll(need & ((1ull << lane) - 1));
            if (!active && take < end) {
                idx = take;
                row = hit_row[idx];
                steps = 0;
                active = true;
            }
            next += __popcll(need);
            if (!__any(active)) break;
            if (active) {
                bool sampled = ix.sa_pow2_shift != 0xffffffffu ? (row & (ix.sa_s - 1)) == 0 : (row % ix.sa_s) == 0;
                if (sampled) {
                    uint32_t j = ix.sa_pow2_shift != 0xffffffffu ? row >> ix.sa_pow2_shift : row / ix.sa_s;
                    hit_ref[idx] = ix.sa_sample[j] + steps;
                    active = false;
                } else {
                    uint32_t blk = row >> kBlockShift, off = row & (kBlockRows - 1);
                    LoadedBlock b = load_block(ix.blocks, blk);
                    uint32_t c = block_code(b, off);
                    if (c == kCodeSentinel) {
                        hit_ref[idx] = steps;
                        active = false;
                    } else {
                        row = less_of(ix, c) + block_rank(b, c, blk, off, ix.sentinel_row);
                        steps++;
                        my_steps++;
                        if (steps > ix.n) {
                            hit_ref[idx] = 0;
                            active = false;
                        }
                    }
                }
            }
        }
    }
    for (int d = 32; d > 0; d >>= 1) my_steps += __shfl_down(my_steps, d);
    if (lane == 0 && my_steps) atomicAdd(lf_steps, my_steps);
}

}

namespace {
__global__ void k_publish(const uint64_t* __restrict__ src, uint64_t* dst, uint32_t n) {
    if (threadIdx.x < n) __hip_atomic_store(dst + threadIdx.x, src[threadIdx.x], __ATOMIC_RELAXED, __HIP_MEMORY_SCOPE_SYSTEM);
}
}

void launch_publish(hipStream_t s, const uint64_t* src, uint64_t* dst_host, uint32_t n) {
    hipLaunchKernelGGL(k_publish, dim3(1), dim3(64), 0, s, src, dst_host, n);
}

void launch_normalise(hipStream_t s, const uint8_t* src, uint8_t* dst, uint64_t begin, uint64_t end) {
    if (end <= begin) return;
    const uint64_t n = end - (begin & ~15ull);
    hipLaunchKernelGGL(k_normalise, dim3(cdiv((n + 15) / 16, 256)), dim3(256), 0, s, src, dst, begin, end);
}
void launch_unpack(hipStream_t s, const uint8_t* packed, uint8_t* dst, uint64_t lo, uint64_t hi) {
    if (hi <= lo) return;
    const uint64_t groups = ((hi + 15) >> 4) - (lo >> 4);
    hipLaunchKernelGGL(k_unpack, dim3((uint32_t)cdiv(groups, 256)), dim3(256), 0, s, packed, dst, lo, hi);
}

void launch_search(hipStream_t s, const DevIndexView& ix, const uint8_t* bases, const uint32_t* read_off, uint32_t r0,
                   uint32_t n_reads, uint32_t max_ns, uint32_t K, uint32_t G, uint32_t* seed_lo, uint32_t* seed_cnt,
                   uint32_t* slow_list, uint32_t* slow_count, uint32_t listed_cap, const uint2* kmer_levels) {
    (void)hipMemsetAsync(slow_count, 0, sizeof(uint32_t), s);
    uint64_t total = (uint64_t)n_reads * 2 * max_ns;
    if (!total) return;
    const bool fast = ix.kmer_tab && total < 0xffffffffull && K >= 16 && K <= 24 && ix.kmer_k >= 12 && ix.kmer_k <= 17 &&
                      K >= ix.kmer_k && K - std::min<uint32_t>(ix.kmer_k, 16) <= 8 && !getenv("MTSV_SEARCH_GENERIC");
    if (!fast) {
        hipLaunchKernelGGL(k_search, dim3(cdiv(total, 256)), dim3(256), 0, s, ix, bases, read_off, r0, n_reads, max_ns, K, G,
                           seed_lo, seed_cnt, kmer_levels);
        return;
    }
    const dim3 grid(std::min<uint32_t>(cdiv(total, 256), 256 * 16));
#define FAST_CASE(KKV)                                                                                                  \
    if (K - KKV > 2)                                                                                                    \
        hipLaunchKernelGGL((k_search_fast<KKV, true>), grid, dim3(256), 0, s, ix, bases, read_off, r0, (uint32_t)total, max_ns, K, G, \
                           seed_lo, seed_cnt, slow_list, slow_count);                                                   \
    else                                                                                                                \
        hipLaunchKernelGGL((k_search_fast<KKV, false>), grid, dim3(256), 0, s, ix, bases, read_off, r0, (uint32_t)total, max_ns, K, G, \
                           seed_lo, seed_cnt, slow_list, slow_count)
    switch (ix.kmer_k) {
    case 12: FAST_CASE(12); break;
    case 13: FAST_CASE(13); break;
    case 14: FAST_CASE(14); break;
    case 15: FAST_CASE(15); break;
    case 17: FAST_CASE(17); break;
    default: FAST_CASE(16); break;
    }
#undef FAST_CASE
    hipLaunchKernelGGL(k_search_listed, dim3(cdiv(std::max<uint32_t>(listed_cap, 1), 256)), dim3(256), 0, s, ix, bases, read_off, r0, max_ns, K, G,
                       slow_list, slow_count, seed_lo, seed_cnt, kmer_levels);
}

void launch_thin(hipStream_t s, const uint8_t* bases, const uint32_t* read_off, uint32_t r0, uint32_t n_reads, double edit_rate,
                 double min_seed, uint32_t max_ns, uint32_t K, uint32_t G, uint64_t max_hits, uint64_t tune, uint32_t* seed_cnt, uint32_t* seed_pre,
                 uint32_t* strand_hits, uint32_t* strand_nseeds, uint32_t* planes, uint32_t plane_words) {
    hipLaunchKernelGGL(k_thin, dim3(cdiv((uint64_t)n_reads * 2, 256)), dim3(256), 0, s, bases, read_off, r0, n_reads, edit_rate,
                       min_seed, max_ns, K, G, max_hits, tune, seed_cnt, seed_pre, strand_hits, strand_nseeds, planes, plane_words);
}

void launch_scan(hipStream_t s, const uint32_t* in, uint32_t n, uint64_t* tile_sums, uint64_t* total, uint32_t* out) {
    uint32_t tiles = cdiv(n ? n : 1, kScanTile);
    hipLaunchKernelGGL(k_scan_tile_sums, dim3(tiles), dim3(kScanThreads), 0, s, in, n, tile_sums);
    hipLaunchKernelGGL(k_scan_sums, dim3(1), dim3(1024), 0, s, tile_sums, tiles, total);
    hipLaunchKernelGGL(k_scan_apply, dim3(tiles), dim3(kScanThreads), 0, s, in, n, tile_sums, total, out);
}
uint32_t scan_tiles(uint32_t n) { return cdiv(n ? n : 1, kScanTile); }

void launch_expand(hipStream_t s, const DevIndexView& ix, uint32_t n_strands, uint32_t max_ns, uint32_t G,
                   const uint32_t* seed_lo, const uint32_t* seed_cnt, const uint32_t* seed_pre, const uint32_t* strand_off,
                   uint32_t* hit_row, uint32_t* hit_ref, uint32_t* hit_q) {
    uint64_t n_slots = (uint64_t)n_strands * max_ns;
    if (!n_slots) return;
    hipLaunchKernelGGL(k_expand, dim3(cdiv(n_slots, 256)), dim3(256), 0, s, ix, n_slots, max_ns, G, seed_lo, seed_cnt, seed_pre,
                       strand_off, hit_row, hit_ref, hit_q);
}

void launch_locate(hipStream_t s, const DevIndexView& ix, uint32_t total_hits_host, const uint32_t* total_hits_dev,
                   const uint32_t* hit_row, uint32_t* hit_ref, unsigned long long* lf_steps) {
    if (!total_hits_host) return;
    uint32_t chunks = cdiv(total_hits_host, kLocateChunk);
    uint32_t blocks = std::min<uint32_t>(cdiv(chunks, 4), 256 * 8);
    hipLaunchKernelGGL(k_locate, dim3(blocks), dim3(256), 0, s, ix, total_hits_dev, hit_row, hit_ref, lf_steps);
}

}
```

mtsv_tools_amd/csrc/k_verify.hip:

```cpp
#include "kernels_common.hpp"

namespace mtsv {

namespace {

typedef short pk16 __attribute__((ext_vector_type(2)));

__device__ inline pk16 pk(int lo, int hi) {
    pk16 r;
    r.x = (short)lo;
    r.y = (short)hi;
    return r;
}
__device__ inline pk16 pk_max(pk16 a, pk16 b) { return __builtin_elementwise_max(a, b); }
__device__ inline int pk_bits(pk16 a) { return __builtin_bit_cast(int, a); }
__device__ inline pk16 pk_from_bits(int u) { return __builtin_bit_cast(pk16, u); }

constexpr uint32_t kGroup = 16;
constexpr uint32_t kRing = 1024;

__device__ inline int row_shr1(int v) { return __builtin_amdgcn_update_dpp(0, v, 0x111, 0xf, 0xf, true); }

__device__ inline uint32_t group_ballot(bool p, uint32_t group) { return (uint32_t)(__ballot(p) >> (group * kGroup)) & 0xffffu; }

// ... 1210 lines not shown
            }
            const uint32_t Wn = c.y - c.x;
            int score = (int)L, best = (int)L;
            const bool swm = BOUND || (LIST && ph == 1);
            uint4 nxt4 = Wn ? fetch_cols(ix, c.x, c.y, strand, 0, swm) : make_uint4(0, 0, 0, 0);
            const uint32_t* lane_tab = &eq_tab[0][0][tid];
            uint32_t j0 = 0;
            uint32_t win_n = 0;
            for (; j0 < Wn; j0 += 16) {
                if (swm) {
                    if (BOUND && best <= (int)ED) break;
                    if (best > 2 * (int)ED && score - (int)(Wn - j0) > 2 * (int)ED) break;
                }
                const uint4 cur = nxt4;
                if (LIST) win_n |= cur.x | cur.y | cur.z | cur.w;
                if (j0 + 16 < Wn) nxt4 = fetch_cols(ix, c.x, c.y, strand, j0 + 16, swm);
                const uint32_t lim = min(16u, Wn - j0);
#pragma unroll
                for (int jj = 0; jj < 16; jj++) {
                    if ((uint32_t)jj < lim) {
                        const uint32_t word = jj < 4 ? cur.x : jj < 8 ? cur.y : jj < 12 ? cur.z : cur.w;
                        const uint32_t tc = (word >> ((jj & 3) * 8)) & 0xffu;
                        const uint32_t* row = lane_tab + tc * (W * 256);
                        uint32_t ph_below = 0, mh_below = 0;
#pragma unroll
                        for (int k = 0; k < W; k++) {
                            const uint32_t Eq = row[k * 256];
                            const uint32_t pv = Pv[k], mv = Mv[k];
                            const uint32_t Xv = Eq | mv;
                            const uint32_t Eqh = k ? (Eq | (mh_below >> 31)) : Eq;
                            const uint32_t Xh = __builtin_amdgcn_bitop3_b32((Eqh & pv) + pv, pv, Eqh, 0xBE);
                            const uint32_t Ph = mv | ~(Xh | pv);
                            const uint32_t Mh = pv & Xh;
                            const uint32_t Phs = k ? __builtin_amdgcn_alignbit(Ph, ph_below, 31) : (Ph << 1);
                            const uint32_t Mhs = k ? __builtin_amdgcn_alignbit(Mh, mh_below, 31) : (Mh << 1);
                            Pv[k] = Mhs | ~(Xv | Phs);
                            Mv[k] = Phs & Xv;
                            ph_below = Ph;
                            mh_below = Mh;
                        }
                        const uint32_t hp = ph_below >> 31, hm = mh_below >> 31;
                        score += (int)hp - (int)hm;
                        best = min(best, score);
                    }
                }
            }
            cols += min(j0, Wn);
            if (LIST ? ph == 1 : (!BOUND || !counted)) {
                verified++;
                wbytes += Wn;
            }
            counted = false;
            const uint32_t ed = (uint32_t)best;
            if (BOUND) {
                if (!thr_wrapped && ed <= ED) {
                    verdict = 1;
                    vg = g;
                    active = false;
                } else if (!thr_wrapped && ed <= 2 * ED) {
                    verdict = 2;
                    vg = g;
                    active = false;
                } else {
                    refuted++;
                    a.cand_status[g] = 1;
                    const uint32_t nxt = a.cand_next[g];
                    if (nxt == 0xffffffffu || nxt >= maxc) active = false;
                    else g = o + nxt;
                }
            } else if (LIST && ph == 1) {
                if (ed > 2 * ED) {
                    if (FUSED) refuted++;
                    a.cand_status[g] = 1;
                    const uint32_t nxt = a.cand_next[g];
                    if (nxt == 0xffffffffu || nxt >= maxc) active = false;
                    else g = o + nxt;
                } else if (ed > ED) {
                    if (FUSED) {
                        verdict = 2;
                    } else {
                        a.next_list[atomicAdd(a.next_count, 1u)] = g | kSweepFlag;
                    }
                    active = false;
                } else {
                    extra_passed++;
                    if (!read_n || !(win_n & 0x04040404u)) {
                        const DevBin bin = ix.bins[c.z];
                        a.out[g] = make_uint4(bin.tax_id, bin.gi, c.x >= bin.start ? c.x - bin.start : 0, ed);
                        a.cand_status[g] = 2;
                        active = false;
                    } else {
                        ph = 2;
                    }
                }
            } else {
            const bool pass = !thr_wrapped && ed <= ED;
            if (pass) {
                const DevBin bin = ix.bins[c.z];
                a.out[g] = make_uint4(bin.tax_id, bin.gi, c.x >= bin.start ? c.x - bin.start : 0, ed);
                a.cand_status[g] = 2;
                active = false;
            } else {
                a.cand_status[g] = 1;
                const uint32_t nxt = a.cand_next[g];
                if (nxt == 0xffffffffu || nxt >= maxc) active = false;
                else {
                    g = o + nxt;
                    if (LIST) ph = 1;
                }
            }
            }
        }
        if (BOUND || FUSED) {
            const unsigned long long pm = BOUND ? __ballot(verdict == 1) : 0ull, um = __ballot(verdict == 2);
            const unsigned long long lower = (1ull << lane) - 1ull;
            if (pm) {
                uint32_t base = 0;
                if (lane == 0) base = atomicAdd(sw_pass_count(a), (uint32_t)__popcll(pm));
                base = __builtin_amdgcn_readfirstlane(base);
                if (verdict == 1) a.pass_list[base + (uint32_t)__popcll(pm & lower)] = vg;
            }
            if (um) {
                uint32_t base = 0;
                if (lane == 0) base = atomicAdd(reinterpret_cast<uint32_t*>(a.counters + a.und_slot), (uint32_t)__popcll(um));
                base = __builtin_amdgcn_readfirstlane(base);
                if (verdict == 2) a.und_list[base + (uint32_t)__popcll(um & lower)] = (FUSED ? g : vg) | kSweepFlag;
            }
        }
    }
    unsigned long long v64 = verified, w64 = wbytes;
    for (int d = 32; d > 0; d >>= 1) {
        v64 += __shfl_down(v64, d);
        w64 += __shfl_down(w64, d);
    }
    if (lane == 0 && v64) {
        atomicAdd(a.n_verified, v64);
        atomicAdd(a.window_bytes, w64);
    }
    if (a.myers_ctr) {
        unsigned long long c64 = cols, r64 = refuted;
        for (int d = 32; d > 0; d >>= 1) {
            c64 += __shfl_down(c64, d);
            r64 += __shfl_down(r64, d);
        }
        unsigned long long e64 = extra_passed;
        for (int d = 32; d > 0; d >>= 1) e64 += __shfl_down(e64, d);
        if (lane == 0) {
            atomicAdd(a.myers_ctr, c64);
            if ((BOUND || FUSED) && r64) atomicAdd(a.myers_ctr + 1, r64);
            if (LIST && e64) atomicAdd(a.myers_ctr + 2, e64);
        }
    }
}

__global__ __launch_bounds__(256) void k_resolve(uint32_t n_strands, int64_t max_candidates, int64_t max_assignments,
                                                 const uint32_t* __restrict__ strand_off,
                                                 const uint32_t* __restrict__ strand_ncand,
                                                 const uint32_t* __restrict__ cand_status, uint4* __restrict__ out,
                                                 uint32_t* __restrict__ strand_nout) {
    const uint32_t rs = blockIdx.x * blockDim.x + threadIdx.x;
    const bool valid = rs < n_strands;
    uint32_t nc = valid ? strand_ncand[rs] : 0;
    uint32_t nout = 0;
    const uint32_t o = nc ? strand_off[rs] : 0;
    if (max_candidates >= 0 && (uint64_t)nc > (uint64_t)max_candidates) nc = (uint32_t)max_candidates;
    constexpr uint32_t kCoop = 32;
    const bool big = nc > kCoop;
    if (nc && !big) {
        for (uint32_t i = 0; i < nc; i++) {
            if (cand_status[o + i] == 2) {
                if (nout != i) out[o + nout] = out[o + i];
                nout++;
                if (max_assignments >= 0 && (uint64_t)nout >= (uint64_t)max_assignments) break;
            }
        }
    }
    const uint32_t lane = lane_id();
    const uint64_t cap = max_assignments < 0 ? ~0ull : (uint64_t)(max_assignments > 1 ? max_assignments : 1);
    for (unsigned long long m = __ballot(big); m; m &= m - 1) {
        const int l = __builtin_ctzll(m);
        const uint32_t o_l = __builtin_amdgcn_readlane(o, l), nc_l = __builtin_amdgcn_readlane(nc, l);
        uint32_t nout_l = 0;
        for (uint32_t base = 0; base < nc_l; base += kWave) {
            const uint32_t i = base + lane;
            const bool pass = i < nc_l && cand_status[o_l + i] == 2;
            uint4 v = make_uint4(0, 0, 0, 0);
            if (pass) v = out[o_l + i];
            const unsigned long long pm = __ballot(pass);
            const uint32_t pos = nout_l + (uint32_t)__popcll(pm & ((1ull << lane) - 1));
            if (pass && (uint64_t)pos < cap) out[o_l + pos] = v;
            nout_l += (uint32_t)__popcll(pm);
            if ((uint64_t)nout_l >= cap) {
                nout_l = (uint32_t)cap;
                break;
            }
        }
        if ((int)lane == l) nout = nout_l;
    }
    if (!valid) return;
    strand_nout[rs] = nout;
}

__global__ __launch_bounds__(256) void k_gather(uint32_t n_strands, uint64_t r0, const uint32_t* __restrict__ strand_off,
                                                const uint32_t* __restrict__ strand_nout,
                                                const uint32_t* __restrict__ out_off, const uint4* __restrict__ out,
                                                DevHit* __restrict__ hits, uint64_t hits_base) {
    uint32_t rs = blockIdx.x * blockDim.x + threadIdx.x;
    if (rs >= n_strands) return;
    uint32_t n = strand_nout[rs];
    if (!n) return;
    uint32_t src = strand_off[rs];
    uint64_t dst = hits_base + out_off[rs];
    for (uint32_t i = 0; i < n; i++) {
        uint4 v = out[src + i];
        DevHit h;
        h.read = r0 + (rs >> 1);
        h.tax_id = v.x;
        h.gi = v.y;
        h.edit = v.w;
        h.strand = rs & 1;
        h.offset = v.z;
        hits[dst + i] = h;
    }
}

}

void launch_evaluate(hipStream_t s, const DevIndexView& ix, const EvalArgs& a_, uint64_t max_items, uint32_t max_len) {
    EvalArgs a = a_;
    a.maxc = rank_bound(a.max_candidates);
#define EVAL_CASE(RR, WW, GG) hipLaunchKernelGGL((k_evaluate<RR, WW, GG>), dim3(std::max<uint32_t>(1, std::min<uint32_t>(cdiv(max_items, 256 / GG), 256 * 8))), dim3(256), 0, s, ix, a)
    if (max_len <= 32) EVAL_CASE(2, false, 16);
    else if (max_len <= 64) EVAL_CASE(4, false, 16);
    else if (max_len <= 80) EVAL_CASE(5, false, 16);
    else if (max_len <= 112) EVAL_CASE(7, false, 16);
    else if (max_len <= 128) EVAL_CASE(8, false, 16);
    else if (max_len <= 160) EVAL_CASE(10, false, 16);
    else if (max_len <= 208) EVAL_CASE(13, false, 16);
    else if (max_len < 254) EVAL_CASE(16, false, 16);
    else if (max_len <= kMaxRegisterReadLen) EVAL_CASE(16, true, 16);
    else throw std::runtime_error("internal: launch_evaluate called for a read beyond the register-resident kernels");
#undef EVAL_CASE
}

uint32_t tiled_groups(uint64_t max_items, uint32_t strip_len) {
    const uint64_t by_mem = std::max<uint64_t>(1, (1ull << 30) / (16ull * 8 * std::max<uint32_t>(strip_len, 1)));
    const uint32_t blocks = (uint32_t)std::max<uint64_t>(1, std::min<uint64_t>(std::min<uint64_t>(cdiv(max_items, 16), 256 * 2), by_mem));
    return blocks * 16;
}

void launch_evaluate_tiled(hipStream_t s, const DevIndexView& ix, const EvalArgs& a_, uint64_t max_items) {
    EvalArgs a = a_;
    a.maxc = rank_bound(a.max_candidates);
    const uint32_t blocks = tiled_groups(max_items, a.strip_len) / 16;
    hipLaunchKernelGGL((k_evaluate<16, true, 16, true>), dim3(blocks), dim3(256), 0, s, ix, a);
}

void launch_sw_pairs(hipStream_t s, const DevIndexView& ix, const EvalArgs& a_, uint64_t max_items_, uint32_t max_len, bool diag, bool top, bool sparse) {
    const uint64_t max_items = sparse ? std::max<uint64_t>(max_items_ / 64, 1024) : max_items_;
    EvalArgs a = a_;
    a.maxc = rank_bound(a.max_candidates);
    if (top) {
#define SW_TOP(RR)                                                                                                       \
    do {                                                                                                                 \
        const uint32_t grid = std::max<uint32_t>(1, std::min<uint32_t>(cdiv(max_items, 32), 256 * kSwTopOcc));           \
        a.claim_shift = 0;                                                                                               \
        while ((1ull << a.claim_shift) < (uint64_t)grid * 16 * 2) a.claim_shift++;                                       \
        hipLaunchKernelGGL((k_sw_pairs<RR, false, true>), dim3(grid), dim3(256), 0, s, ix, a);                           \
    } while (0)
        if (max_len <= 64) SW_TOP(2);
        else if (max_len <= 96) SW_TOP(3);
        else if (max_len <= 128) SW_TOP(4);
        else if (max_len <= 160) SW_TOP(5);
        else if (max_len <= 208) SW_TOP(7);
        else SW_TOP(8);
#undef SW_TOP
        return;
    }
#define SW_CASE(RR)                                                                                                      \
    do {                                                                                                                 \
        const uint32_t grid = std::max<uint32_t>(1, std::min<uint32_t>(cdiv(max_items, 32), 256 * ((RR) > 10 ? 3 : kSwOcc))); \
        a.claim_shift = 0;                                                                                               \
        while ((1ull << a.claim_shift) < (uint64_t)grid * 16 * 2) a.claim_shift++;                                       \
        if (diag) hipLaunchKernelGGL((k_sw_pairs<RR, true>), dim3(grid), dim3(256), 0, s, ix, a);                        \
        else hipLaunchKernelGGL((k_sw_pairs<RR, false>), dim3(grid), dim3(256), 0, s, ix, a);                            \
    } while (0)
    if (max_len <= 64) SW_CASE(4);
    else if (max_len <= 96) SW_CASE(6);
    else if (max_len <= 128) SW_CASE(8);
    else if (max_len <= 160) SW_CASE(10);
    else if (max_len <= 208) SW_CASE(13);
    else SW_CASE(16);
#undef SW_CASE
}

void launch_sw_diag(hipStream_t s, const DevIndexView& ix, const EvalArgs& a, uint64_t max_items, uint32_t max_len,
                    uint32_t* sweep_list, uint32_t sweep_slot) {
    const uint32_t grid = std::max<uint32_t>(16, std::min<uint32_t>(cdiv(max_items, 16 * 32), 256 * 6));
    if (max_len <= 128) hipLaunchKernelGGL(k_sw_diag<2>, dim3(grid), dim3(256), 0, s, ix, a, sweep_list, sweep_slot);
    else if (max_len <= 192) hipLaunchKernelGGL(k_sw_diag<3>, dim3(grid), dim3(256), 0, s, ix, a, sweep_list, sweep_slot);
    else hipLaunchKernelGGL(k_sw_diag<4>, dim3(grid), dim3(256), 0, s, ix, a, sweep_list, sweep_slot);
}

void launch_edit_myers(hipStream_t s, const DevIndexView& ix, const EvalArgs& a_, uint64_t max_items, uint32_t max_len,
                       int mode) {
    EvalArgs a = a_;
    a.maxc = rank_bound(a.max_candidates);
    if (!a.planes || a.plane_words != myers_words(max_len)) throw std::runtime_error("internal: k_edit_myers needs the pass's read planes");
    uint32_t blocks = std::max<uint32_t>(16, std::min<uint32_t>(cdiv(max_items, 4096), 256 * 5));
    const uint32_t W = myers_words(max_len);
#define MYERS_CASE(WW)                                                                                   \
    do {                                                                                                 \
        if (mode == MY_LIST) hipLaunchKernelGGL((k_edit_myers<WW, MY_LIST>), dim3(blocks), dim3(256), 0, s, ix, a);        \
        else if (mode == MY_FUSED) hipLaunchKernelGGL((k_edit_myers<WW, MY_FUSED>), dim3(blocks), dim3(256), 0, s, ix, a); \
        else if (mode == MY_BOUND) hipLaunchKernelGGL((k_edit_myers<WW, MY_BOUND>), dim3(blocks), dim3(256), 0, s, ix, a); \
        else hipLaunchKernelGGL((k_edit_myers<WW, MY_CHAIN>), dim3(blocks), dim3(256), 0, s, ix, a);                      \
    } while (0)
    if (W == 2) MYERS_CASE(2);
    else if (W == 3) MYERS_CASE(3);
    else if (W == 4) MYERS_CASE(4);
    else if (W == 5) MYERS_CASE(5);
    else if (W == 6) MYERS_CASE(6);
    else if (W == 7) MYERS_CASE(7);
    else MYERS_CASE(8);
#undef MYERS_CASE
}

void launch_resolve(hipStream_t s, uint32_t n_strands, int64_t max_candidates, int64_t max_assignments,
                    const uint32_t* strand_off, const uint32_t* strand_ncand, const uint32_t* cand_status, uint4* out,
                    uint32_t* strand_nout) {
    hipLaunchKernelGGL(k_resolve, dim3(cdiv(n_strands, 256)), dim3(256), 0, s, n_strands, max_candidates, max_assignments,
                       strand_off, strand_ncand, cand_status, out, strand_nout);
}

void launch_gather(hipStream_t s, uint32_t n_strands, uint64_t r0, const uint32_t* strand_off, const uint32_t* strand_nout,
                   const uint32_t* out_off, const uint4* out, DevHit* hits, uint64_t hits_base) {
    hipLaunchKernelGGL(k_gather, dim3(cdiv(n_strands, 256)), dim3(256), 0, s, n_strands, r0, strand_off, strand_nout,
                       out_off, out, hits, hits_base);
}

}
```

mtsv_tools_amd/csrc/kernels.hpp:

```cpp
#pragma once
#include <algorithm>

#include "dev_layout.hpp"

namespace mtsv {

struct DevHit {
    uint64_t read;
    uint32_t tax_id;
    uint32_t gi;
    uint32_t edit;
    uint8_t strand;
    uint8_t pad[3];
    uint64_t offset;
};
static_assert(sizeof(DevHit) == 32, "DevHit must match mtsv_hit");

constexpr uint32_t kCtrVerified = 4, kCtrWindowBytes = 5, kCtrSwCursor = 8, kCtrPassCount = 9, kCtrSwCellPairs = 14;
constexpr uint32_t kCtrHeavyWalk = 23, kCtrHeavyTicket = 24;

struct EvalArgs {
    const uint8_t* bases;
    const uint32_t* read_off;
    uint32_t r0;
    double edit_rate;
    int64_t max_candidates;
    const uint32_t* strand_off;
    const uint4* cand;
    const uint32_t* cand_next;
    uint32_t* cand_status;
    const uint32_t* worklist;
    const uint32_t* wl_count;
    uint32_t* wl_cursor;
    uint32_t wl_reverse = 0;
    uint64_t* counters = nullptr;
    uint32_t wl_count_slot = 0;
    uint4* out;
    unsigned long long* n_verified;
    unsigned long long* window_bytes;
    unsigned long long* sw_columns = nullptr;
    uint32_t* pass_list = nullptr;
    uint32_t* pass_count = nullptr;
    uint32_t* next_list = nullptr;
    uint32_t* next_count = nullptr;
    unsigned long long* myers_ctr = nullptr;
    uint32_t* und_list = nullptr;
    uint32_t und_slot = 0;
    uint2* strip = nullptr;
    uint32_t strip_len = 0;
    const uint32_t* planes = nullptr;
    uint32_t plane_words = 0;
    uint32_t maxc = 0xffffffffu;
    uint32_t claim_shift = 0;
};

inline uint32_t myers_words(uint32_t max_len) { return std::min(std::max((max_len + 31) / 32, 2u), 8u); }

constexpr uint32_t kMaxRegisterReadLen = 256;
constexpr uint32_t kMaxReadLen = 32767;

void launch_publish(hipStream_t s, const uint64_t* src, uint64_t* dst_host, uint32_t n);
void launch_normalise(hipStream_t s, const uint8_t* src, uint8_t* dst, uint64_t begin, uint64_t end);
void launch_unpack(hipStream_t s, const uint8_t* packed, uint8_t* dst, uint64_t lo, uint64_t hi);
void launch_search(hipStream_t s, const DevIndexView& ix, const uint8_t* bases, const uint32_t* read_off, uint32_t r0,
                   uint32_t n_reads, uint32_t max_ns, uint32_t K, uint32_t G, uint32_t* seed_lo, uint32_t* seed_cnt,
                   uint32_t* slow_list, uint32_t* slow_count, uint32_t listed_cap, const uint2* kmer_levels);
void launch_thin(hipStream_t s, const uint8_t* bases, const uint32_t* read_off, uint32_t r0, uint32_t n_reads, double edit_rate,
                 double min_seed, uint32_t max_ns, uint32_t K, uint32_t G, uint64_t max_hits, uint64_t tune, uint32_t* seed_cnt, uint32_t* seed_pre,
                 uint32_t* strand_hits, uint32_t* strand_nseeds, uint32_t* planes, uint32_t plane_words);
void launch_scan(hipStream_t s, const uint32_t* in, uint32_t n, uint64_t* tile_sums, uint64_t* total, uint32_t* out);
uint32_t scan_tiles(uint32_t n);
void launch_expand(hipStream_t s, const DevIndexView& ix, uint32_t n_strands, uint32_t max_ns, uint32_t G,
                   const uint32_t* seed_lo, const uint32_t* seed_cnt, const uint32_t* seed_pre, const uint32_t* strand_off,
                   uint32_t* hit_row, uint32_t* hit_ref, uint32_t* hit_q);
void launch_locate(hipStream_t s, const DevIndexView& ix, uint32_t total_hits_host, const uint32_t* total_hits_dev,
                   const uint32_t* hit_row, uint32_t* hit_ref, unsigned long long* lf_steps);
void launch_coalesce(hipStream_t s, const DevIndexView& ix, const uint32_t* read_off, uint32_t r0, uint32_t n_strands,
                     int64_t max_candidates, const uint32_t* strand_off,
                     const uint32_t* strand_nseeds, const uint32_t* hit_ref, const uint32_t* hit_q, uint64_t* hit_key,
                     uint64_t* cand_tmp, uint4* cand, uint32_t* cand_next, uint32_t* cand_status,
                     uint32_t* strand_ncand, uint32_t* worklist, uint32_t* heavy_list, uint64_t* counters);
void launch_evaluate(hipStream_t s, const DevIndexView& ix, const EvalArgs& a, uint64_t max_items, uint32_t max_len);
void launch_evaluate_tiled(hipStream_t s, const DevIndexView& ix, const EvalArgs& a, uint64_t max_items);
uint32_t tiled_groups(uint64_t max_items, uint32_t strip_len);
void launch_max_window(hipStream_t s, uint32_t n_strands, const uint32_t* strand_off, const uint32_t* strand_ncand,
                       const uint4* cand, unsigned long long* out);
void launch_edit_myers(hipStream_t s, const DevIndexView& ix, const EvalArgs& a, uint64_t max_items, uint32_t max_len,
                       int mode = 0);
void launch_sw_pairs(hipStream_t s, const DevIndexView& ix, const EvalArgs& a, uint64_t max_items, uint32_t max_len,
                     bool diag = true, bool top = false, bool sparse = false);
void launch_sw_diag(hipStream_t s, const DevIndexView& ix, const EvalArgs& a, uint64_t max_items, uint32_t max_len,
                    uint32_t* sweep_list, uint32_t sweep_slot);
void launch_resolve(hipStream_t s, uint32_t n_strands, int64_t max_candidates, int64_t max_assignments,
                    const uint32_t* strand_off, const uint32_t* strand_ncand, const uint32_t* cand_status, uint4* out,
                    uint32_t* strand_nout);
void launch_gather(hipStream_t s, uint32_t n_strands, uint64_t r0, const uint32_t* strand_off, const uint32_t* strand_nout,
                   const uint32_t* out_off, const uint4* out, DevHit* hits, uint64_t hits_base);
constexpr uint32_t kReportDenseTaxa = 4095;
constexpr uint32_t kReportHashSlots = 4096;
void launch_report(hipStream_t s, uint32_t n_reads, const uint32_t* strand_nout, const uint32_t* out_off, const DevHit* hits,
                   const uint32_t* taxa, uint32_t n_taxa, bool dense, uint32_t hash_slots, uint64_t* counts, uint64_t* total_reads,
                   uint64_t* n_global);
void launch_match(hipStream_t s, uint32_t n_reads, const uint32_t* strand_nout, uint64_t first_bit, uint64_t* words, uint64_t* n_matched);

}
```

Before: 405.1 million.

## Serialize multi-lane verify phase, fuse counter clears, size tail rounds from list

Adds a host-side turn lock so that only one lane at a time runs the verify stage, ordered by first read. When several lanes are active, the Myers grid is capped at three workgroups per CU. The separate small hipMemsetAsync counter resets are replaced by a single masked clear kernel, and redundant resets are skipped when a counter is already known to be zero. Later rounds size the SW/Myers launches from the published undecided-list count and skip empty tails. The catch is an extra host sync after the bound pass and less overlap between lanes in the verify stage.

After: 425.0 million, median of 6. +4.9%, better.

```diff
diff --git a/include/mtsv_amd.h b/include/mtsv_amd.h
--- a/include/mtsv_amd.h
+++ b/include/mtsv_amd.h
@@ -74,6 +74,9 @@
     float edit_ms;
     uint64_t myers_columns;
     uint64_t n_sw_bound_refuted;
+    uint64_t verify_turns;
+    uint64_t verify_lanes_max;
+    uint64_t myers_grid_max;
 } mtsv_batch_stats;
 
 const char *mtsv_last_error(void);
diff --git a/mtsv_tools_amd/_lib.py b/mtsv_tools_amd/_lib.py
--- a/mtsv_tools_amd/_lib.py
+++ b/mtsv_tools_amd/_lib.py
@@ -43,7 +43,8 @@
                 ("window_bytes", C.c_uint64), ("n_hits", C.c_uint64), ("n_passes", C.c_uint64),
                 ("n_rounds", C.c_uint64), ("n_lanes", C.c_uint64), ("sw_cell_pairs", C.c_uint64), ("sw_prefilter_ms", C.c_float),
                 ("sw_sweep_ms", C.c_float), ("n_sw_passed", C.c_uint64), ("sw_diag_ms", C.c_float), ("sw_bound_ms", C.c_float),
-                ("edit_ms", C.c_float), ("myers_columns", C.c_uint64), ("n_sw_bound_refuted", C.c_uint64)]
+                ("edit_ms", C.c_float), ("myers_columns", C.c_uint64), ("n_sw_bound_refuted", C.c_uint64),
+                ("verify_turns", C.c_uint64), ("verify_lanes_max", C.c_uint64), ("myers_grid_max", C.c_uint64)]
 
     def as_dict(self):
         d = {n: (float(getattr(self, n)) if t is C.c_float else int(getattr(self, n))) for n, t in self._fields_[1:]}
diff --git a/mtsv_tools_amd/csrc/batch.hip b/mtsv_tools_amd/csrc/batch.hip
--- a/mtsv_tools_amd/csrc/batch.hip
+++ b/mtsv_tools_amd/csrc/batch.hip
@@ -86,6 +86,7 @@
 
 int g_default_verify_mode = MTSV_VERIFY_REFERENCE;
 
+constexpr uint32_t kMyersWgsPerCuLanes = 3;
 constexpr uint64_t kLaneMinReads = 32768;
 constexpr uint64_t kChunkMaxReads = 4ull << 20;
 
@@ -139,6 +140,18 @@
     if (const char* e = getenv("MTSV_SW_FUSED")) sw_fused = atoi(e) != 0;
     verify_mode = g_default_verify_mode;
     if (const char* e = getenv("MTSV_VERIFY")) verify_mode = !strcmp(e, "edit_first") ? 1 : 0;
+    if (!parent) {
+        myers_wgs_per_cu = n_lanes > 1 ? kMyersWgsPerCuLanes : kMyersWgsPerCuMax;
+        if (const char* e = getenv("MTSV_MYERS_WGS_PER_CU")) myers_wgs_per_cu = (uint32_t)std::max(1, std::min((int)kMyersWgsPerCuMax, atoi(e)));
+        verify_turn.on = n_lanes > 1;
+        if (const char* e = getenv("MTSV_VERIFY_TURN")) verify_turn.on = verify_turn.on && atoi(e) != 0;
+        if (const char* e = getenv("MTSV_TAIL_FROM_LIST")) tail_from_list = atoi(e) != 0;
+        if (const char* e = getenv("MTSV_FUSED_CLEAR")) fused_clear = atoi(e) != 0;
+    } else {
+        myers_wgs_per_cu = parent->myers_wgs_per_cu;
+        tail_from_list = parent->tail_from_list;
+        fused_clear = parent->fused_clear;
+    }
     for (auto& e : ev) HIP_CHECK(hipEventCreate(&e));
     for (int k = 1; k < n_lanes; k++) {
         extra.emplace_back(new Batch(ix, di, ws_reads, 0, hit_cap_user, this));
@@ -212,6 +225,33 @@
     alloc_hit_workspace();
 }
 
+void Batch::VerifyTurn::enter(uint64_t first_read, const Batch* lane) {
+    std::unique_lock<std::mutex> lk(mu);
+    if (on) {
+        const std::pair<uint64_t, const Batch*> me{first_read, lane};
+        waiting.push_back(me);
+        cv.wait(lk, [&] { return !held && *std::min_element(waiting.begin(), waiting.end()) == me; });
+        waiting.erase(std::find(waiting.begin(), waiting.end(), me));
+        held = true;
+        taken++;
+    }
+    max_in_verify = std::max(max_in_verify, ++in_verify);
+}
+
+void Batch::VerifyTurn::leave() {
+    {
+        std::lock_guard<std::mutex> lk(mu);
+        in_verify--;
+        held = false;
+    }
+    cv.notify_all();
+}
+
+void Batch::VerifyTurn::note_grid(uint32_t blocks) {
+    std::lock_guard<std::mutex> lk(mu);
+    myers_grid_max = std::max<uint64_t>(myers_grid_max, blocks);
+}
+
 void Batch::upload(const uint8_t* bases, const uint64_t* read_off, uint64_t n) {
     if (n > max_reads) throw std::runtime_error("arg: batch holds more reads than the workspace was created for");
     const uint64_t first = n ? read_off[0] : 0;
@@ -244,6 +284,7 @@
     sw_passed_acc = 0;
     n_hits_total = 0;
     HIP_CHECK(hipMemsetAsync(d_counters, 0, kCounters * sizeof(uint64_t), stream));
+    ctr22_zero = true;
     HIP_CHECK(hipEventRecord(ev[8], stream));
 }
 
@@ -280,6 +321,10 @@
     lanes_used = 1;
     staged_valid = false;
     run_t0 = now_s();
+    {
+        std::lock_guard<std::mutex> lk(verify_turn.mu);
+        verify_turn.taken = verify_turn.max_in_verify = verify_turn.myers_grid_max = 0;
+    }
     reset_lane();
     for (auto& l : extra) {
         l->verify_mode = verify_mode;
@@ -341,6 +386,9 @@
     for (int s = 0; s < MTSV_N_STAGES; s++) stats.stage_ms[s] = stage_acc[s];
     stats.n_reads = n_reads;
     stats.n_lanes = lanes_used;
+    stats.verify_turns = verify_turn.taken;
+    stats.verify_lanes_max = verify_turn.max_in_verify;
+    stats.myers_grid_max = verify_turn.myers_grid_max;
     total_hits = 0;
     for (auto& sg : segments) total_hits += sg.count;
     stats.n_hits = total_hits;
@@ -556,7 +604,9 @@
             dev_alloc(&d_seed_pre, want, &dummy);
             seed_cap = want;
         }
-        const bool myers_pass = !tiled && pass_max_len <= 253 && (verify_mode == 1 || (sw_pairs && hit_cap < 0x80000000ull));
+        const bool edit_first_path = !tiled && verify_mode == 1 && pass_max_len <= 253;
+        const bool rounds_path = !tiled && !edit_first_path && sw_pairs && pass_max_len <= 253 && hit_cap < 0x80000000ull;
+        const bool myers_pass = edit_first_path || rounds_path;
         const uint32_t plane_words = myers_pass ? myers_words(pass_max_len) : 0;
         if ((uint64_t)nr * 3 * plane_words > plane_cap) {
             (void)hipFree(d_planes);
@@ -568,7 +618,9 @@
         }
         HIP_CHECK(hipEventRecord(ev[0], stream));
         const uint32_t listed_cap = (uint32_t)std::min<uint64_t>(slots, std::max<uint64_t>(4096, (uint64_t)((double)slots * listed_share)));
-        launch_search(stream, v, sb, so, (uint32_t)r0, nr, max_ns, K, G, d_seed_lo, d_seed_cnt, d_seed_pre, (uint32_t*)(d_counters + 22), listed_cap, di->d_kmer_levels);
+        launch_search(stream, v, sb, so, (uint32_t)r0, nr, max_ns, K, G, d_seed_lo, d_seed_cnt, d_seed_pre, (uint32_t*)(d_counters + 22), listed_cap, di->d_kmer_levels,
+                      fused_clear && ctr22_zero);
+        ctr22_zero = false;
         HIP_CHECK(hipEventRecord(ev[1], stream));
         if (max_ns)
             launch_thin(stream, sb, so, (uint32_t)r0, nr, p.edit_rate, p.min_seed, max_ns, K, G, p.max_hits, p.tune_max_hits, d_seed_cnt,
@@ -612,13 +664,24 @@
             launch_locate(stream, v, (uint32_t)total_hits, d_strand_off + nstr, d_hit_row, d_hit_ref,
                           (unsigned long long*)(d_counters + 2));
         HIP_CHECK(hipEventRecord(ev[4], stream));
-        HIP_CHECK(hipMemsetAsync(d_counters + 1, 0, 8, stream));
-        HIP_CHECK(hipMemsetAsync(d_counters + 7, 0, 8, stream));
-        HIP_CHECK(hipMemsetAsync(d_counters + 15, 0, 8, stream));
+        if (fused_clear) {
+            uint64_t mask = 1ull << 1 | 1ull << 7 | 1ull << 15 | 1ull << kCtrHeavyTicket | 1ull << 22;
+            if (rounds_path) mask |= 1ull << 8 | 1ull << 9 | 1ull << 10 | 1ull << 11 | 1ull << 17 | 1ull << 18;
+            launch_clear_counters(stream, d_counters, mask);
+            ctr22_zero = true;
+        } else {
+            HIP_CHECK(hipMemsetAsync(d_counters + 1, 0, 8, stream));
+            HIP_CHECK(hipMemsetAsync(d_counters + 7, 0, 8, stream));
+            HIP_CHECK(hipMemsetAsync(d_counters + 15, 0, 8, stream));
+        }
         launch_coalesce(stream, v, so, (uint32_t)r0, nstr, p.max_candidates, d_strand_off,
                         d_strand_nseeds, d_hit_ref, d_hit_q, d_hit_key, d_cand_tmp, d_cand, d_cand_next,
-                        d_cand_status, d_strand_ncand, d_worklist, d_heavy_list, d_counters);
+                        d_cand_status, d_strand_ncand, d_worklist, d_heavy_list, d_counters, fused_clear);
         HIP_CHECK(hipEventRecord(ev[5], stream));
+        Batch* const root = parent ? parent : this;
+        VerifyTurn::Guard turn;
+        if (total_hits) turn.take(root->verify_turn, read_base + r0, this);
+        const uint32_t R = root->myers_wgs_per_cu;
         {
             EvalArgs a;
             a.bases = sb;
@@ -657,9 +720,9 @@
                 a.strip = d_strip;
                 a.strip_len = strip_len;
                 launch_evaluate_tiled(stream, v, a, total_hits);
-            } else if (verify_mode == 1 && pass_max_len <= 253) {
-                launch_edit_myers(stream, v, a, total_hits, pass_max_len);
-            } else if (sw_pairs && pass_max_len <= 253 && hit_cap < 0x80000000ull) {
+            } else if (edit_first_path) {
+                root->verify_turn.note_grid(launch_edit_myers(stream, v, a, total_hits, pass_max_len, 0, R));
+            } else if (rounds_path) {
                 const bool fused = sw_bound && sw_fused;
                 uint32_t* pass_list = (uint32_t*)d_hit_key;
                 uint32_t* sweep_list = (uint32_t*)d_hit_key + hit_cap;
@@ -669,8 +732,14 @@
                 uint64_t items = total_hits;
                 for (uint32_t round = 0;; round++) {
                     uint64_t* next_slot = d_counters + 11 + (round & 1);
-                    HIP_CHECK(hipMemsetAsync(d_counters + 8, 0, 3 * sizeof(uint64_t), stream));
-                    HIP_CHECK(hipMemsetAsync(next_slot, 0, sizeof(uint64_t), stream));
+                    if (!fused_clear) {
+                        HIP_CHECK(hipMemsetAsync(d_counters + 8, 0, 3 * sizeof(uint64_t), stream));
+                        HIP_CHECK(hipMemsetAsync(next_slot, 0, sizeof(uint64_t), stream));
+                    } else if (round) {
+                        launch_clear_counters(stream, d_counters, 1ull << 8 | 1ull << 9 | 1ull << 10 | 1ull << (11 + (round & 1)));
+                    }
+                    uint64_t tail_items = items;
+                    bool tail_listed = tail_from_list && round > 0;
                     EvalArgs sw = a;
                     sw.worklist = wl;
                     sw.wl_count = wl_count;
@@ -695,18 +764,24 @@
                         sw.wl_reverse = 0;
                     }
                     if (round == 0 && sw_bound) {
-                        HIP_CHECK(hipMemsetAsync(d_counters + 17, 0, 2 * sizeof(uint64_t), stream));
+                        if (!fused_clear) HIP_CHECK(hipMemsetAsync(d_counters + 17, 0, 2 * sizeof(uint64_t), stream));
                         EvalArgs bd = sw;
                         bd.wl_count = (const uint32_t*)(d_counters + sw.wl_count_slot);
                         bd.wl_cursor = (uint32_t*)(d_counters + 18);
                         bd.und_list = (uint32_t*)d_hit_row;
                         bd.und_slot = 17;
                         bd.myers_ctr = (unsigned long long*)(d_counters + 19);
-                        launch_edit_myers(stream, v, bd, items, pass_max_len, fused ? 3 : 2);
+                        root->verify_turn.note_grid(launch_edit_myers(stream, v, bd, items, pass_max_len, fused ? 3 : 2, R));
                         HIP_CHECK(hipEventRecord(ev[13], stream));
                         sw.worklist = bd.und_list;
                         sw.wl_count_slot = 17;
                         sw.wl_reverse = 0;
+                        if (fused && tail_from_list) {
+                            launch_publish(stream, d_counters + 17, h_counters + 17, 1);
+                            HIP_CHECK(hipStreamSynchronize(stream));
+                            tail_items = h_counters[17] & 0xffffffffull;
+                            tail_listed = true;
+                        }
                     } else if (round == 0 && sw_diag && sw_prepass && sw_top) {
                         HIP_CHECK(hipMemsetAsync(d_counters + 17, 0, sizeof(uint64_t), stream));
                         sw.und_list = (uint32_t*)d_hit_row;
@@ -716,7 +791,8 @@
                         sw.worklist = sw.und_list;
                         sw.wl_count_slot = 17;
                     }
-                    launch_sw_pairs(stream, v, sw, items, pass_max_len, sw_diag, false, round == 0 && sw_bound);
+                    const bool tail_empty = tail_listed && tail_items == 0;
+                    if (!tail_empty) launch_sw_pairs(stream, v, sw, tail_items, pass_max_len, sw_diag, false, round == 0 && sw_bound && !tail_listed);
 #ifdef MTSV_SW_HIST
                     {
                         static uint32_t hh[768];
@@ -739,11 +815,16 @@
                     my.next_list = next_lists[round & 1];
                     my.next_count = (uint32_t*)next_slot;
                     my.myers_ctr = (unsigned long long*)(d_counters + 19);
-                    launch_edit_myers(stream, v, my, items, pass_max_len, 1);
+                    if (!tail_empty) root->verify_turn.note_grid(launch_edit_myers(stream, v, my, tail_items, pass_max_len, 1, R, tail_listed));
                     if (round == 0) HIP_CHECK(hipEventRecord(ev[14], stream));
-                    launch_publish(stream, next_slot, h_counters + 11, 1);
-                    launch_publish(stream, d_counters + 9, h_counters + 9, 1);
-                    HIP_CHECK(hipStreamSynchronize(stream));
+                    if (tail_empty) {
+                        h_counters[9] = h_counters[11] = 0;
+                        if (round == 0) HIP_CHECK(hipEventSynchronize(ev[14]));
+                    } else {
+                        launch_publish(stream, next_slot, h_counters + 11, 1);
+                        launch_publish(stream, d_counters + 9, h_counters + 9, 1);
+                        HIP_CHECK(hipStreamSynchronize(stream));
+                    }
                     sw_passed_acc += h_counters[9] & 0xffffffffull;
                     if (round == 0) {
                         float ms = 0;
@@ -772,6 +853,7 @@
                     wl_count = (const uint32_t*)next_slot;
                     items = n_next;
                 }
+                turn.release();
             } else {
                 launch_evaluate(stream, v, a, total_hits, pass_max_len);
             }
@@ -785,6 +867,7 @@
             launch_publish(stream, d_counters, h_counters, 8);
             HIP_CHECK(hipStreamSynchronize(stream));
             total_out = h_counters[6];
+            turn.release();
         }
         if (n_hits_total + total_out > hits_cap) {
             uint64_t ncap = std::max(hits_cap * 2, n_hits_total + total_out);
@@ -824,6 +907,7 @@
         }
         HIP_CHECK(hipStreamSynchronize(stream));
         HIP_CHECK(hipGetLastError());
+        turn.release();
         if (mf.mode != MTSV_MATCH_OFF) {
             float ms = 0;
             HIP_CHECK(hipEventElapsedTime(&ms, match_ev[0], match_ev[1]));
diff --git a/mtsv_tools_amd/csrc/batch.hpp b/mtsv_tools_amd/csrc/batch.hpp
--- a/mtsv_tools_amd/csrc/batch.hpp
+++ b/mtsv_tools_amd/csrc/batch.hpp
@@ -1,4 +1,5 @@
 #pragma once
+#include <condition_variable>
 #include <memory>
 #include <mutex>
 #include <vector>
@@ -81,6 +82,38 @@
     bool sw_fused = true;
     bool sw_prepass = true;
     bool sw_pairs = true;
+    uint32_t myers_wgs_per_cu = kMyersWgsPerCuMax;
+    bool tail_from_list = true;
+    bool fused_clear = true;
+    bool ctr22_zero = false;
+    struct VerifyTurn {
+        bool on = false;
+        std::mutex mu;
+        std::condition_variable cv;
+        bool held = false;
+        std::vector<std::pair<uint64_t, const Batch*>> waiting;
+        uint64_t taken = 0, in_verify = 0, max_in_verify = 0, myers_grid_max = 0;
+        void enter(uint64_t first_read, const Batch* lane);
+        void leave();
+        void note_grid(uint32_t blocks);
+        struct Guard {
+            VerifyTurn* t = nullptr;
+            Guard() = default;
+            Guard(const Guard&) = delete;
+            Guard& operator=(const Guard&) = delete;
+            ~Guard() { release(); }
+            void take(VerifyTurn& turn, uint64_t first_read, const Batch* lane) {
+                if (t) return;
+                turn.enter(first_read, lane);
+                t = &turn;
+            }
+            void release() {
+                if (t) t->leave();
+                t = nullptr;
+            }
+        };
+    };
+    VerifyTurn verify_turn;
     int verify_mode = 0;
     uint64_t n_reads = 0;
     uint64_t n_hits_total = 0;
diff --git a/mtsv_tools_amd/csrc/k_coalesce.hip b/mtsv_tools_amd/csrc/k_coalesce.hip
--- a/mtsv_tools_amd/csrc/k_coalesce.hip
+++ b/mtsv_tools_amd/csrc/k_coalesce.hip
@@ -850,7 +850,8 @@
                      int64_t max_candidates, const uint32_t* strand_off,
                      const uint32_t* strand_nseeds, const uint32_t* hit_ref, const uint32_t* hit_q, uint64_t* hit_key,
                      uint64_t* cand_tmp, uint4* cand, uint32_t* cand_next, uint32_t* cand_status,
-                     uint32_t* strand_ncand, uint32_t* worklist, uint32_t* heavy_list, uint64_t* counters) {
+                     uint32_t* strand_ncand, uint32_t* worklist, uint32_t* heavy_list, uint64_t* counters,
+                     bool ticket_is_zero) {
     uint32_t* wl_count = reinterpret_cast<uint32_t*>(counters + 1);
     uint32_t* heavy_count = wl_count + 1;
     unsigned long long* n_cand_total = reinterpret_cast<unsigned long long*>(counters + 3);
@@ -897,7 +898,7 @@
     if (serial_walk || ix.n_bins >= 0x80000000u) {
         hipLaunchKernelGGL((k_coalesce_heavy<kHeavyKeysSmall, false>), hgrid, dim3(256), 0, s, ix, a, heavy_list, n_strands, heavy_count);
     } else {
-        (void)hipMemsetAsync(counters + kCtrHeavyTicket, 0, sizeof(uint64_t), s);
+        if (!ticket_is_zero) (void)hipMemsetAsync(counters + kCtrHeavyTicket, 0, sizeof(uint64_t), s);
         hipLaunchKernelGGL((k_coalesce_heavy<kHeavyKeysSmall, true>), hgrid, dim3(256), 0, s, ix, a, heavy_list, n_strands, heavy_count);
     }
     hipLaunchKernelGGL((k_coalesce_heavy<kHeavyKeys, false>), dim3(std::min<uint32_t>(hgrid.x, 512)), dim3(256), 0, s, ix, a, heavy_list, n_strands, heavy_count);
diff --git a/mtsv_tools_amd/csrc/k_seed.hip b/mtsv_tools_amd/csrc/k_seed.hip
--- a/mtsv_tools_amd/csrc/k_seed.hip
+++ b/mtsv_tools_amd/csrc/k_seed.hip
@@ -694,10 +694,17 @@
 __global__ void k_publish(const uint64_t* __restrict__ src, uint64_t* dst, uint32_t n) {
     if (threadIdx.x < n) __hip_atomic_store(dst + threadIdx.x, src[threadIdx.x], __ATOMIC_RELAXED, __HIP_MEMORY_SCOPE_SYSTEM);
 }
+__global__ void k_clear_counters(uint64_t* counters, uint64_t mask) {
+    if ((mask >> threadIdx.x) & 1) counters[threadIdx.x] = 0;
+}
 }
 
 void launch_publish(hipStream_t s, const uint64_t* src, uint64_t* dst_host, uint32_t n) {
     hipLaunchKernelGGL(k_publish, dim3(1), dim3(64), 0, s, src, dst_host, n);
+}
+
+void launch_clear_counters(hipStream_t s, uint64_t* counters, uint64_t mask) {
+    if (mask) hipLaunchKernelGGL(k_clear_counters, dim3(1), dim3(64), 0, s, counters, mask);
 }
 
 void launch_normalise(hipStream_t s, const uint8_t* src, uint8_t* dst, uint64_t begin, uint64_t end) {
@@ -713,8 +720,9 @@
 
 void launch_search(hipStream_t s, const DevIndexView& ix, const uint8_t* bases, const uint32_t* read_off, uint32_t r0,
                    uint32_t n_reads, uint32_t max_ns, uint32_t K, uint32_t G, uint32_t* seed_lo, uint32_t* seed_cnt,
-                   uint32_t* slow_list, uint32_t* slow_count, uint32_t listed_cap, const uint2* kmer_levels) {
-    (void)hipMemsetAsync(slow_count, 0, sizeof(uint32_t), s);
+                   uint32_t* slow_list, uint32_t* slow_count, uint32_t listed_cap, const uint2* kmer_levels,
+                   bool count_is_zero) {
+    if (!count_is_zero) (void)hipMemsetAsync(slow_count, 0, sizeof(uint32_t), s);
     uint64_t total = (uint64_t)n_reads * 2 * max_ns;
     if (!total) return;
     const bool fast = ix.kmer_tab && total < 0xffffffffull && K >= 16 && K <= 24 && ix.kmer_k >= 12 && ix.kmer_k <= 17 &&
diff --git a/mtsv_tools_amd/csrc/k_verify.hip b/mtsv_tools_amd/csrc/k_verify.hip
--- a/mtsv_tools_amd/csrc/k_verify.hip
+++ b/mtsv_tools_amd/csrc/k_verify.hip
@@ -1536,12 +1536,13 @@
     else hipLaunchKernelGGL(k_sw_diag<4>, dim3(grid), dim3(256), 0, s, ix, a, sweep_list, sweep_slot);
 }
 
-void launch_edit_myers(hipStream_t s, const DevIndexView& ix, const EvalArgs& a_, uint64_t max_items, uint32_t max_len,
-                       int mode) {
+uint32_t launch_edit_myers(hipStream_t s, const DevIndexView& ix, const EvalArgs& a_, uint64_t max_items, uint32_t max_len,
+                           int mode, uint32_t wgs_per_cu, bool listed) {
     EvalArgs a = a_;
     a.maxc = rank_bound(a.max_candidates);
     if (!a.planes || a.plane_words != myers_words(max_len)) throw std::runtime_error("internal: k_edit_myers needs the pass's read planes");
-    uint32_t blocks = std::max<uint32_t>(16, std::min<uint32_t>(cdiv(max_items, 4096), 256 * 5));
+    const uint32_t resident = 256 * std::max<uint32_t>(1, std::min<uint32_t>(wgs_per_cu, kMyersWgsPerCuMax));
+    uint32_t blocks = std::max<uint32_t>(16, std::min<uint32_t>(cdiv(max_items, listed ? 256 : 4096), resident));
     const uint32_t W = myers_words(max_len);
 #define MYERS_CASE(WW)                                                                                   \
     do {                                                                                                 \
@@ -1558,6 +1559,7 @@
     else if (W == 7) MYERS_CASE(7);
     else MYERS_CASE(8);
 #undef MYERS_CASE
+    return blocks;
 }
 
 void launch_resolve(hipStream_t s, uint32_t n_strands, int64_t max_candidates, int64_t max_assignments,
diff --git a/mtsv_tools_amd/csrc/kernels.hpp b/mtsv_tools_amd/csrc/kernels.hpp
--- a/mtsv_tools_amd/csrc/kernels.hpp
+++ b/mtsv_tools_amd/csrc/kernels.hpp
@@ -60,11 +60,13 @@
 constexpr uint32_t kMaxReadLen = 32767;
 
 void launch_publish(hipStream_t s, const uint64_t* src, uint64_t* dst_host, uint32_t n);
+void launch_clear_counters(hipStream_t s, uint64_t* counters, uint64_t mask);
 void launch_normalise(hipStream_t s, const uint8_t* src, uint8_t* dst, uint64_t begin, uint64_t end);
 void launch_unpack(hipStream_t s, const uint8_t* packed, uint8_t* dst, uint64_t lo, uint64_t hi);
 void launch_search(hipStream_t s, const DevIndexView& ix, const uint8_t* bases, const uint32_t* read_off, uint32_t r0,
                    uint32_t n_reads, uint32_t max_ns, uint32_t K, uint32_t G, uint32_t* seed_lo, uint32_t* seed_cnt,
-                   uint32_t* slow_list, uint32_t* slow_count, uint32_t listed_cap, const uint2* kmer_levels);
+                   uint32_t* slow_list, uint32_t* slow_count, uint32_t listed_cap, const uint2* kmer_levels,
+                   bool count_is_zero = false);
 void launch_thin(hipStream_t s, const uint8_t* bases, const uint32_t* read_off, uint32_t r0, uint32_t n_reads, double edit_rate,
                  double min_seed, uint32_t max_ns, uint32_t K, uint32_t G, uint64_t max_hits, uint64_t tune, uint32_t* seed_cnt, uint32_t* seed_pre,
                  uint32_t* strand_hits, uint32_t* strand_nseeds, uint32_t* planes, uint32_t plane_words);
@@ -79,14 +81,16 @@
                      int64_t max_candidates, const uint32_t* strand_off,
                      const uint32_t* strand_nseeds, const uint32_t* hit_ref, const uint32_t* hit_q, uint64_t* hit_key,
                      uint64_t* cand_tmp, uint4* cand, uint32_t* cand_next, uint32_t* cand_status,
-                     uint32_t* strand_ncand, uint32_t* worklist, uint32_t* heavy_list, uint64_t* counters);
+                     uint32_t* strand_ncand, uint32_t* worklist, uint32_t* heavy_list, uint64_t* counters,
+                     bool ticket_is_zero = false);
 void launch_evaluate(hipStream_t s, const DevIndexView& ix, const EvalArgs& a, uint64_t max_items, uint32_t max_len);
 void launch_evaluate_tiled(hipStream_t s, const DevIndexView& ix, const EvalArgs& a, uint64_t max_items);
 uint32_t tiled_groups(uint64_t max_items, uint32_t strip_len);
 void launch_max_window(hipStream_t s, uint32_t n_strands, const uint32_t* strand_off, const uint32_t* strand_ncand,
                        const uint4* cand, unsigned long long* out);
-void launch_edit_myers(hipStream_t s, const DevIndexView& ix, const EvalArgs& a, uint64_t max_items, uint32_t max_len,
-                       int mode = 0);
+constexpr uint32_t kMyersWgsPerCuMax = 5;
+uint32_t launch_edit_myers(hipStream_t s, const DevIndexView& ix, const EvalArgs& a, uint64_t max_items, uint32_t max_len,
+                           int mode = 0, uint32_t wgs_per_cu = kMyersWgsPerCuMax, bool listed = false);
 void launch_sw_pairs(hipStream_t s, const DevIndexView& ix, const EvalArgs& a, uint64_t max_items, uint32_t max_len,
                      bool diag = true, bool top = false, bool sparse = false);
 void launch_sw_diag(hipStream_t s, const DevIndexView& ix, const EvalArgs& a, uint64_t max_items, uint32_t max_len,
```
